# bbc/vc2-reference

Measured on AMD Instinct MI355X. Metric: Mpixels/s encode+decode, UHD-1 10-bit HQ_ConstQ, higher is better.
Workload: dtype int32; 1 GPU; BASELINE cfg2: UHD-1 3840x2160 4:2:2 10-bit HQ_ConstQ DD97 depth 4, -u 1 -a 2 -q 16 -S 2; streams=1, parallelism=frame-parallel x1, no collective

## Files before the change

include/vc2hip.h:

```cpp
#ifndef VC2HIP_H
#define VC2HIP_H

#include <stddef.h>
#include <stdint.h>

#ifdef __cplusplus
extern "C" {
#endif
#if defined(__GNUC__)
#pragma GCC visibility push(default)
#endif

typedef struct vc2hip_ctx vc2hip_ctx;

enum { VC2HIP_DD97 = 0, VC2HIP_LEGALL = 1, VC2HIP_DD137 = 2, VC2HIP_HAAR0 = 3,
       VC2HIP_HAAR1 = 4, VC2HIP_FIDELITY = 5, VC2HIP_DAUB97 = 6 };
enum { VC2HIP_CF444 = 0, VC2HIP_CF422 = 1, VC2HIP_CF420 = 2 };
enum { VC2HIP_HQ_CONSTQ = 0, VC2HIP_HQ_CBR = 1, VC2HIP_LD = 2, VC2HIP_HQ_CAPPED = 3 };
#define VC2HIP_CAP_Q_TOP 115

enum {
  VC2HIP_OK = 0,
  VC2HIP_EINVAL = -1,
  VC2HIP_EQINDEX = -2,
  VC2HIP_ESCALAR = -3,
  VC2HIP_ECBR_TOOBIG = -4,
  VC2HIP_ECBR_LEN = -5,
  VC2HIP_ECBR_WRONG = -6,
  VC2HIP_EBOUNDED = -7,
  VC2HIP_ELD_TOOBIG = -8,
  VC2HIP_ECAP = -9,
  VC2HIP_ESTREAM = -10,
  VC2HIP_ECODE32 = -11,
  VC2HIP_ESYNTAX = -12,
  VC2HIP_EHIP = -100
};

int vc2hip_create(int device, vc2hip_ctx **out);
#define VC2HIP_FLAG_STORE32         0x001u
#define VC2HIP_FLAG_NO_STREAM       0x002u
#define VC2HIP_FLAG_NO_PAIR         0x004u
#define VC2HIP_FLAG_NO_BANDPLANES   0x008u
#define VC2HIP_FLAG_NO_HEADS        0x010u
#define VC2HIP_FLAG_NO_CBR_INDEX    0x020u
#define VC2HIP_FLAG_GENERIC_DWT     0x040u
#define VC2HIP_FLAG_SINGLE_PASS_VBR 0x080u
#define VC2HIP_FLAG_CBR_GENERAL     0x100u
#define VC2HIP_FLAG_LD_DIAGONALS    0x200u
#define VC2HIP_FLAG_PLANES8_ALWAYS  0x400u
#define VC2HIP_FLAG_PLANES8_NEVER   0x800u
#define VC2HIP_FLAG_TWO_PASS_VBR    0x1000u
#define VC2HIP_FLAG_CAP_GENERAL     0x2000u
int vc2hip_create_with_flags(int device, unsigned flags, vc2hip_ctx **out);
int vc2hip_create_on_stream(int device, void *hip_stream, vc2hip_ctx **out);
int vc2hip_create_on_stream_with_flags(int device, void *hip_stream, unsigned flags, vc2hip_ctx **out);
void vc2hip_destroy(vc2hip_ctx *ctx);
const char *vc2hip_last_error(const vc2hip_ctx *ctx);
const char *vc2hip_error_string(int code);
int vc2hip_sync(vc2hip_ctx *ctx);

int vc2hip_padded_size(int size, int depth);
int vc2hip_slice_size_is_valid(int depth, int len_luma, int len_chroma, int n_size);
int vc2hip_quant_matrix(int kernel, int depth, int32_t *out);
int vc2hip_slice_bytes(int y_slices, int x_slices, int total_bytes, int scalar, int32_t *out);

int vc2hip_dwt_forward(vc2hip_ctx *ctx, const int32_t *in, int h, int w, int kernel, int depth,
                       int32_t *out);
int vc2hip_dwt_inverse(vc2hip_ctx *ctx, const int32_t *in, int ph, int pw, int kernel, int depth,
                       int32_t *out, int h, int w);
int vc2hip_quantise_np(vc2hip_ctx *ctx, const int32_t *coef, int ph, int pw, int depth,
                       const int32_t *qidx, int ys, int xs, const int32_t *qmatrix, int32_t *out);
int vc2hip_dequantise_np(vc2hip_ctx *ctx, const int32_t *q, int ph, int pw, int depth,
                         const int32_t *qidx, int ys, int xs, const int32_t *qmatrix, int32_t *out);
int vc2hip_dequantise_ld(vc2hip_ctx *ctx, const int32_t *q, int ph, int pw, int depth,
                         const int32_t *qidx, int ys, int xs, const int32_t *qmatrix, int32_t *out);

int vc2hip_quantise_ld(vc2hip_ctx *ctx, const int32_t *coef, int ph, int pw, int depth,
                       const int32_t *qidx, int ys, int xs, const int32_t *qmatrix, int32_t *out);

typedef struct {
  int luma_h, luma_w;
  int chroma_h, chroma_w;
  int depth;
  int y_slices, x_slices;
} vc2hip_geom;

int vc2hip_hq_pack(vc2hip_ctx *ctx, const int32_t *y, const int32_t *u, const int32_t *v,
                   const vc2hip_geom *g, const int32_t *qidx, int prefix, int scalar,
                   const int32_t *cbr_slice_bytes, uint8_t *out, size_t cap, size_t *out_len);
int vc2hip_hq_unpack(vc2hip_ctx *ctx, const uint8_t *in, size_t len, const vc2hip_geom *g,
                     int prefix, int scalar, int32_t *y, int32_t *u, int32_t *v, int32_t *qidx,
                     size_t *consumed);
int vc2hip_ld_unpack(vc2hip_ctx *ctx, const uint8_t *in, size_t len, const vc2hip_geom *g,
                     const int32_t *slice_bytes, int32_t *y, int32_t *u, int32_t *v,
                     int32_t *qidx, size_t *consumed);
int vc2hip_ld_pack(vc2hip_ctx *ctx, const int32_t *y, const int32_t *u, const int32_t *v,
                   const vc2hip_geom *g, const int32_t *qidx, const int32_t *slice_bytes,
                   uint8_t *out, size_t cap, size_t *out_len);
int vc2hip_ld_qindices(vc2hip_ctx *ctx, const int32_t *y, const int32_t *u, const int32_t *v,
                       const vc2hip_geom *g, const int32_t *qmatrix, const int32_t *slice_bytes,
                       int32_t *qidx);
int vc2hip_cbr_qindices(vc2hip_ctx *ctx, const int32_t *y, const int32_t *u, const int32_t *v,
                        const vc2hip_geom *g, const int32_t *qmatrix, const int32_t *slice_bytes,
                        int scalar, int32_t *qidx);

// ... 55 lines not shown
  int packing;
  int little_endian, lsb_justified;
  size_t pitch[2];
  size_t plane_offset[2];
  size_t picture_stride;
} vc2hip_packed_format;
int vc2hip_set_packed_format(vc2hip_ctx *ctx, const vc2hip_packed_format *pf);
size_t vc2hip_packed_picture_bytes(const vc2hip_picture_format *fmt, const vc2hip_packed_format *pf);
int vc2hip_encode_batch_dev(vc2hip_ctx *ctx, const void *d_raw, int n,
                            const vc2hip_picture_format *fmt, const vc2hip_coding_params *cp,
                            void *d_payload, size_t payload_stride, uint64_t *d_lens);
int vc2hip_decode_batch_dev(vc2hip_ctx *ctx, const void *d_payload, size_t payload_stride,
                            const uint64_t *d_lens, int n, const vc2hip_picture_format *fmt,
                            const vc2hip_coding_params *cp, void *d_raw_out);
int vc2hip_decode_reduced_batch_dev(vc2hip_ctx *ctx, const void *d_payload, size_t payload_stride,
                                    const uint64_t *d_lens, int n, const vc2hip_picture_format *fmt,
                                    const vc2hip_coding_params *cp, int drop_levels, void *d_raw_out);
int vc2hip_encode_recon_batch_dev(vc2hip_ctx *ctx, const void *d_raw, int n,
                                  const vc2hip_picture_format *fmt, const vc2hip_coding_params *cp,
                                  void *d_payload, size_t payload_stride, uint64_t *d_lens,
                                  void *d_recon, uint64_t *d_sse, int32_t *d_qidx);
int vc2hip_encode_fields_batch_dev(vc2hip_ctx *ctx, const void *d_frames, int n_frames,
                                   const vc2hip_picture_format *frame_fmt, int top_field_first,
                                   const vc2hip_coding_params *cp, void *d_payload, size_t payload_stride,
                                   uint64_t *d_lens);
int vc2hip_decode_fields_batch_dev(vc2hip_ctx *ctx, const void *d_payload, size_t payload_stride,
                                   const uint64_t *d_lens, int n_frames, const vc2hip_picture_format *frame_fmt,
                                   int top_field_first, const vc2hip_coding_params *cp, void *d_frames_out);

typedef struct {
  int major_version;
  uint32_t first_picture_number;
  uint32_t prev_parse_offset;
  int end_of_sequence;
} vc2hip_stream_params;

int vc2hip_picture_header(const vc2hip_coding_params *cp, int major_version, uint32_t picture_number,
                          uint8_t *out, size_t cap, size_t *len);
int vc2hip_stream_write_dev(vc2hip_ctx *ctx, const void *d_payload, size_t payload_stride, const uint64_t *d_lens, int n,
                            const vc2hip_coding_params *cp, const vc2hip_stream_params *sp,
                            uint8_t *d_stream, size_t cap, uint64_t *d_stream_len);
int vc2hip_stream_write_fragments_dev(vc2hip_ctx *ctx, const void *d_payload, size_t payload_stride,
                                      const uint64_t *d_lens, int n, const vc2hip_coding_params *cp,
                                      const vc2hip_stream_params *sp, int fragment_length,
                                      uint8_t *d_stream, size_t cap, uint64_t *d_stream_len,
                                      uint64_t *d_unit_offsets, size_t unit_cap, uint64_t *d_unit_count);
int vc2hip_stream_read_dev(vc2hip_ctx *ctx, const uint8_t *d_stream, size_t len, int n,
                           const vc2hip_coding_params *cp, const vc2hip_stream_params *sp,
                           void *d_payload, size_t payload_stride, uint64_t *d_lens,
                           uint32_t *d_picture_numbers, uint64_t *d_consumed);

int vc2hip_band_plane_bits(const vc2hip_ctx *ctx);

#define VC2HIP_DWT_TILE   0
#define VC2HIP_DWT_FAST   1
#define VC2HIP_DWT_STREAM 2
#define VC2HIP_DWT_PAIR   3
#define VC2HIP_DWT_PLANE  4
typedef struct {
  int inverse;
  int level;
  int levels;
  int family;
  int edge;
  int store_bits;
  int segments;
  int tail;
  int small_gather;
  int pictures;
  int band_planes;
} vc2hip_dwt_launch;
int vc2hip_dwt_launches(const vc2hip_ctx *ctx, vc2hip_dwt_launch *out, int cap);

int vc2hip_profile_enable(vc2hip_ctx *ctx, int on);
int vc2hip_profile_only(vc2hip_ctx *ctx, const char *name);
int vc2hip_profile_count(vc2hip_ctx *ctx);
int vc2hip_profile_get(vc2hip_ctx *ctx, int i, const char **name, int *launches, double *total_ms);
int vc2hip_profile_reset(vc2hip_ctx *ctx);

#if defined(__GNUC__)
#pragma GCC visibility pop
#endif
#ifdef __cplusplus
}
#endif
#endif
```

vc2-reference_amd/csrc/vc2hip_api.hip:

```cpp
#include <math.h>
#include <stdio.h>
#include <stdlib.h>
#include <string.h>

#include <algorithm>
#include <string>
#include <map>
#include <mutex>
#include <utility>
#include <vector>

#include "vc2hip_internal.h"

void vc2_upload_tables_slices(const QuantTables &t, hipStream_t s);
int vc2_halo_x(int kernel);
int vc2_halo_y(int kernel);
void vc2_upload_vlc_lut(hipStream_t s);
void vc2_upload_unpack_lut(hipStream_t s);
bool vc2_slice_index_supported(int prefix, int scalar);
size_t vc2_pack_lds_bytes(int prefix, int scalar);
int vc2_pack_image_mode(int prefix, int scalar);
void vc2_upload_tables_fast(const QuantTables &t, hipStream_t s);
bool vc2_fast_level_applicable(LevelParams &p);
int vc2_launch_forward_fast(Launcher &L, int kernel, bool first, const LevelParams &p, int n, bool store16, hipStream_t s);
// ... 86 lines not shown
#endif
}
void vc2_prof_break(Launcher &L) { (void)L; }

struct Buf {
  void *p = nullptr;
  size_t cap = 0;
};
enum { B_RAW, B_STORE, B_STOREW, B_LL0, B_LLW, B_QIDX, B_SLOTS, B_SIZES, B_OFFS, B_LENS, B_PAYLOAD,
       B_INDEX, B_PLANE, B_PLANE2, B_CBRB, B_CBRO, B_QM, B_UNITS, B_SEGS,
       B_FRAGS, B_FRAGPIC, B_FRAGJUMP,
       B_RSTORE, B_RSTOREW,
       B_PLANE_QM,
       B_CAPTAB,
       B_PKIN, B_PKOUT,
       B_COUNT };

struct vc2hip_ctx {
  int device = 0;
  hipStream_t stream = nullptr;
  bool own_stream = false;
  bool follows_caller = false;
  unsigned *d_err = nullptr;
  unsigned *h_err = nullptr;
  Buf buf[B_COUNT];
  Launcher L;
  std::string err;
  int cbr_key[5] = {-1, -1, -1, -1, -1};
  uint64_t cbr_total = 0;
  int plane_qm_key[2] = {-1, -1};
  int debug_skip = 0;
  bool two_pass_vbr = true;
  bool force_two_pass_vbr = false;
#ifndef VC2_ONE_PASS_MIN_PICTURES
#define VC2_ONE_PASS_MIN_PICTURES 112
#endif
  bool force_generic = false;
  bool allow_store16 = true;
  bool allow_planes = true;
  int planes8_mode = 0;
  bool planes8_on = false;
  unsigned long long *d_stat = nullptr;
  unsigned long long *h_stat = nullptr;
  hipEvent_t stat_ev = nullptr;
  bool stat_pending = false, stat_was8 = false, stat_seen = false;
  int stat_n = 0;
  int stat_n_total = 0;
  int last_plane_bits = 0;
  std::vector<vc2hip_dwt_launch> dwt_rec;
  bool dwt_rec_stale = true;
  double stat_samples = 0;
  int ld_batch = 1;
  bool allow_heads = true;
  bool allow_cbr_index = true;
  bool allow_stream = true;
  bool allow_pair = true;
  bool cbr_general = false;
  bool cap_general = false;
  bool ld_diagonals = false;
  unsigned flags = 0;
  std::vector<vc2hip_ctx *> lanes;
  bool in_split = false;
  hipEvent_t fork_ev = nullptr;
  std::vector<hipEvent_t> join_ev;
  bool lanes_pending = false;
  struct Range { const uint8_t *lo, *hi; };
  enum { LANE_RANGES = 5 };
  struct LaneUse { Range r[LANE_RANGES], w[LANE_RANGES]; bool valid = false; };
  std::vector<LaneUse> lane_use;
  std::vector<ProfEntry> merged;
  struct Flight {
    vc2hip_ctx *lane = nullptr;
    bool open = false, encode = false;
    uint8_t *payload = nullptr;
    size_t cap = 0;
    unsigned long long *h_len = nullptr;
  };
  Flight flight[VC2HIP_MAX_INFLIGHT];
  int flight_next = 0;
  vc2hip_sample_layout layout = {};
  bool has_layout = false, layout_bypass = false;
  vc2hip_packed_format packed = {};
  bool has_packed = false;
};

static const char *code_text(int code) {
  switch (code) {
    case VC2HIP_OK: return "ok";
    case VC2HIP_EINVAL: return "invalid argument";
    case VC2HIP_EQINDEX: return "quantization index exceeds maximum implemented value.";
    case VC2HIP_ESCALAR: return "Slice scalar is too small, consider using a larger slice scalar.";
    case VC2HIP_ECBR_TOOBIG: return "SliceIO, HQ CBR mode: Too many bytes for the slice";
    case VC2HIP_ECBR_LEN: return "Slice component length exceeds 1 byte when divided by slice size scalar. See above for suggestions to prevent this.";
    case VC2HIP_ECBR_WRONG: return "SliceIO, HQ CBR mode: Wrong number of bytes for a slice";
    case VC2HIP_EBOUNDED: return "Attempt to write beyond end of bounded write";
    case VC2HIP_ELD_TOOBIG: return "SliceIO, LD mode: Too many bytes for the U and V slices";
    case VC2HIP_ECAP: return "output buffer too small";
    case VC2HIP_ESTREAM: return "truncated or malformed slice data";
    case VC2HIP_ECODE32: return "quantised coefficient magnitude exceeds 65534 (outside the 32-bit exp-Golomb code domain)";
    case VC2HIP_ESYNTAX: return "VC-2 stream syntax error";
    case VC2HIP_EHIP: return "HIP runtime error";
  }
  return "unknown error";
}
extern "C" const char *vc2hip_error_string(int code) { return code_text(code); }

// ... 68 lines not shown
  const int n = ys * xs;
  int num = total_bytes / scalar - 4 * n, den = n;
  const int g = gcd_i(num, den);
  if (g) { num /= g; den /= g; }
  const int ratio = num / den, rem = num - ratio * den;
  int residue = 0;
  for (int i = 0; i < n; ++i) {
    residue += rem;
    if (residue < den) out[i] = ratio * scalar + 4;
    else { out[i] = (ratio + 1) * scalar + 4; residue -= den; }
  }
  return 0;
}
static void make_tables(QuantTables &t) {
  for (int q = 0; q < 120; ++q) {
    const uint64_t base = 1ull << (q / 4);
    uint64_t f;
    switch (q % 4) {
      case 0: f = 4 * base; break;
      case 1: f = (503829 * base + 52958) / 105917; break;
      case 2: f = (665857 * base + 58854) / 117708; break;
      default: f = (440253 * base + 32722) / 65444; break;
    }
    t.qf[q] = (int32_t)(uint32_t)f;
    t.off[q] = q == 0 ? 1 : (q == 1 ? 2 : (int32_t)(((uint32_t)t.qf[q] + 1u)) / 2);
    t.magic[q] = 0;
    t.shift[q] = 0;
    if (t.qf[q] > 1) {
      const uint64_t d = (uint64_t)t.qf[q];
      int l = 0;
      while ((1ull << l) < d) ++l;
      t.magic[q] = (uint32_t)((((1ull << l) - d) << 32) / d + 1);
      t.shift[q] = l - 1;
    }
    const double r = 4.0 / (double)(uint32_t)t.qf[q];
    float up = (float)r;
    if ((double)up < r) up = nextafterf(up, INFINITY);
    t.inv4[q] = up;
  }
}

static int create_common(int device, hipStream_t stream, bool own, vc2hip_ctx **out, unsigned flags = 0) {
  if (!out) return VC2HIP_EINVAL;
  *out = nullptr;
  int n = 0;
  if (hipGetDeviceCount(&n) != hipSuccess || device < 0 || device >= n) return VC2HIP_EHIP;
  vc2hip_ctx *c = new vc2hip_ctx;
  c->device = device;
#ifdef VC2HIP_ABLATE
  {
    static const struct { const char *name; unsigned flag; } env[] = {
      {"VC2HIP_STORE32", VC2HIP_FLAG_STORE32}, {"VC2HIP_NO_STREAM", VC2HIP_FLAG_NO_STREAM}, {"VC2HIP_NO_PAIR", VC2HIP_FLAG_NO_PAIR},
      {"VC2HIP_NO_BANDPLANES", VC2HIP_FLAG_NO_BANDPLANES}, {"VC2HIP_NO_HEADS", VC2HIP_FLAG_NO_HEADS},
      {"VC2HIP_NO_CBR_INDEX", VC2HIP_FLAG_NO_CBR_INDEX}, {"VC2HIP_GENERIC_DWT", VC2HIP_FLAG_GENERIC_DWT},
      {"VC2HIP_SINGLE_PASS_VBR", VC2HIP_FLAG_SINGLE_PASS_VBR}, {"VC2HIP_TWO_PASS_VBR", VC2HIP_FLAG_TWO_PASS_VBR}, {"VC2HIP_CBR_GENERAL", VC2HIP_FLAG_CBR_GENERAL}, {"VC2HIP_CAP_GENERAL", VC2HIP_FLAG_CAP_GENERAL},
      {"VC2HIP_PLANES8_ALWAYS", VC2HIP_FLAG_PLANES8_ALWAYS}, {"VC2HIP_PLANES8_NEVER", VC2HIP_FLAG_PLANES8_NEVER}};
    for (const auto &e : env) { const char *v = getenv(e.name); if (v && v[0] == '1') flags |= e.flag; }
    { const char *v = getenv("VC2HIP_LD_ROWS"); if (v && v[0] == '0') flags |= VC2HIP_FLAG_LD_DIAGONALS; }
    { const char *e = getenv("VC2HIP_DEBUG_SKIP"); c->debug_skip = e ? atoi(e) : 0; }
  }
#endif
  c->force_generic = (flags & VC2HIP_FLAG_GENERIC_DWT) != 0;
  c->allow_store16 = !(flags & VC2HIP_FLAG_STORE32);
  c->allow_stream = !(flags & VC2HIP_FLAG_NO_STREAM);
  c->allow_pair = !(flags & VC2HIP_FLAG_NO_PAIR);
  c->allow_planes = !(flags & VC2HIP_FLAG_NO_BANDPLANES);
  c->planes8_mode = (flags & VC2HIP_FLAG_PLANES8_NEVER) ? 2 : (flags & VC2HIP_FLAG_PLANES8_ALWAYS) ? 1 : 0;
  c->allow_heads = !(flags & VC2HIP_FLAG_NO_HEADS);
  c->allow_cbr_index = !(flags & VC2HIP_FLAG_NO_CBR_INDEX);
  c->two_pass_vbr = !(flags & VC2HIP_FLAG_SINGLE_PASS_VBR);
  c->force_two_pass_vbr = (flags & VC2HIP_FLAG_TWO_PASS_VBR) != 0;
  c->cbr_general = (flags & VC2HIP_FLAG_CBR_GENERAL) != 0;
  c->cap_general = (flags & VC2HIP_FLAG_CAP_GENERAL) != 0;
  c->ld_diagonals = (flags & VC2HIP_FLAG_LD_DIAGONALS) != 0;
  c->flags = flags;
  if (hipSetDevice(device) != hipSuccess) { delete c; return VC2HIP_EHIP; }
  if (own) { if (hipStreamCreateWithFlags(&stream, hipStreamNonBlocking) != hipSuccess) { delete c; return VC2HIP_EHIP; } }
  c->stream = stream;
  c->own_stream = own;
  c->follows_caller = !own;
  if (hipMalloc((void **)&c->d_err, 256 + 4096) != hipSuccess ||
     
      hipHostMalloc((void **)&c->h_err, VC2_ERRBLK_COPY) != hipSuccess ||
      hipMalloc((void **)&c->d_stat, 64) != hipSuccess || hipHostMalloc((void **)&c->h_stat, 64 * 8) != hipSuccess ||
      hipEventCreateWithFlags(&c->stat_ev, hipEventDisableTiming) != hipSuccess) { delete c; return VC2HIP_EHIP; }
  (void)hipMemsetAsync(c->d_stat, 0, 64, c->stream);
  (void)hipMemsetAsync(c->d_err, 0, sizeof(unsigned), c->stream);
  QuantTables t;
  make_tables(t);
  vc2_upload_tables(t, c->stream);
  vc2_upload_tables_slices(t, c->stream);
  vc2_upload_tables_fast(t, c->stream);
  vc2_upload_tables_pair(t, c->stream);
  vc2_upload_tables_stream(t, c->stream);
  vc2_upload_tables_recon(t, c->stream);
  vc2_upload_vlc_lut(c->stream);
  vc2_upload_unpack_lut(c->stream);
  if (hipStreamSynchronize(c->stream) != hipSuccess) { delete c; return VC2HIP_EHIP; }
  *out = c;
  return VC2HIP_OK;
}
extern "C" int vc2hip_create(int device, vc2hip_ctx **out) { return create_common(device, nullptr, true, out); }
extern "C" int vc2hip_create_with_flags(int device, unsigned flags, vc2hip_ctx **out) { return create_common(device, nullptr, true, out, flags); }
extern "C" int vc2hip_create_on_stream(int device, void *s, vc2hip_ctx **out) { return create_common(device, (hipStream_t)s, false, out); }
extern "C" int vc2hip_create_on_stream_with_flags(int device, void *s, unsigned flags, vc2hip_ctx **out) {
  return create_common(device, (hipStream_t)s, false, out, flags);
}
extern "C" void vc2hip_destroy(vc2hip_ctx *c) {
  if (!c) return;
  (void)hipSetDevice(c->device);
  (void)hipStreamSynchronize(c->stream);
  for (vc2hip_ctx *l : c->lanes) if (l != c) vc2hip_destroy(l);
  for (auto &f : c->flight) { if (f.lane) vc2hip_destroy(f.lane); if (f.h_len) (void)hipHostFree(f.h_len); }
  for (hipEvent_t e : c->join_ev) (void)hipEventDestroy(e);
  if (c->fork_ev) (void)hipEventDestroy(c->fork_ev);
  c->L.collect();
  for (auto e : c->L.pool) (void)hipEventDestroy(e);
  for (auto &b : c->buf) if (b.p) (void)hipFree(b.p);
  if (c->d_err) (void)hipFree(c->d_err);
  if (c->h_err) (void)hipHostFree(c->h_err);
  if (c->h_stat) (void)hipHostFree(c->h_stat);
// ... 440 lines not shown
      const size_t e = (size_t)(g.c[c].ph >> l) * (g.c[c].pw >> l);
      ll.p[l][c] = (char *)base + off * elem_bytes;
      ll.w[l][c] = wide ? wide + off : nullptr;
      ll.stride[l][c] = (long long)e;
      off += (e * n + 7) & ~(size_t)7;
    }
}
static void ll_layout(const Geom &g, int n, int32_t *base, LLPlanes &ll) { ll_layout(g, n, base, 4, nullptr, ll); }

static void record_dwt(vc2hip_ctx *c, bool inverse, int level, int levels, int family, bool edge, bool s16, int segments, int tail,
                       bool small_gather, int n, int band_planes = 0) {
  if (c->dwt_rec_stale) { c->dwt_rec.clear(); c->dwt_rec_stale = false; }
  vc2hip_dwt_launch r;
  r.inverse = inverse; r.level = level; r.levels = levels; r.family = family; r.edge = edge; r.store_bits = s16 ? 16 : 32;
  r.segments = segments; r.tail = tail; r.small_gather = small_gather; r.pictures = n; r.band_planes = band_planes;
  c->dwt_rec.push_back(r);
}

static int band_plane_bits(const LevelParams &p) {
  for (int k = 0; k < 3; ++k) if (p.bp_base[k] >= 0) return p.bp8 ? 8 : 16;
  return 0;
}

static void fill_level(LevelParams &p, const Geom &g, int level, int kernel, const int32_t *qm) {
  const int D = g.depth, Lv = D - level;
  p.band = 3 * (Lv - 1) + 1;
  p.ys = g.ys; p.xs = g.xs; p.slice_coefs = g.slice_coefs;
  const int hx = vc2_halo_x(kernel), hy = vc2_halo_y(kernel);
  for (int c = 0; c < 3; ++c) {
    const CompGeom &cg = g.c[c];
    p.in_h[c] = cg.ph >> level; p.in_w[c] = cg.pw >> level;
    p.pic_h[c] = cg.h; p.pic_w[c] = cg.w;
    p.coef_off[c] = cg.coef_off;
    p.rec_stride[c] = g.slice_coefs;
    if (cg.ph == 0) { p.tiles_x[c] = p.tiles_y[c] = 0; p.fh[c] = p.fw[c] = 2; p.tsy[c] = p.tsx[c] = 1; continue; }
    p.fh[c] = cg.sh >> level; p.fw[c] = cg.sw >> level;
    int tsy = 1, tsx = 1;
    while (tsy * 2 * p.fh[c] <= 64 && tsy * 2 <= g.ys) tsy *= 2;
    while (tsx * 2 * p.fw[c] <= 128 && tsx * 2 <= g.xs) tsx *= 2;
    while ((size_t)(tsy * p.fh[c] + 2 * hy) * (tsx * p.fw[c] + 2 * hx) * 4 > 150 * 1024) {
      if (tsx > 1) tsx /= 2; else if (tsy > 1) tsy /= 2; else break;
    }
    p.tsy[c] = tsy; p.tsx[c] = tsx;
    p.tiles_y[c] = (g.ys + tsy - 1) / tsy;
    p.tiles_x[c] = (g.xs + tsx - 1) / tsx;
    p.band_n[c] = (p.fh[c] / 2) * (p.fw[c] / 2);
    p.band_off[c] = p.band_n[c];
  }
  for (int b = 0; b < 3 * D + 1; ++b) p.qmatrix[b] = qm ? qm[b] : 0;
}

static int run_forward(vc2hip_ctx *c, const Geom &g, int kernel, int n, const void *const src[3],
                       const RawPlane src_l[3], bool src_raw, const vc2hip_picture_format *f,
                       void *store, const LLPlanes &ll, bool s16 = false, int32_t *store_wide = nullptr) {
  auto level_params = [&](LevelParams &p, int level) {
    memset(&p, 0, sizeof p);
    fill_level(p, g, level, kernel, nullptr);
    p.store = store; p.store_stride = (long long)g.ys * g.xs * g.slice_coefs;
    p.store_wide = store_wide;
    p.err = c->d_err;
    p.ll_to_store = (level == g.depth - 1);
    const bool first = (level == 0) && src_raw;
    for (int k = 0; k < 3; ++k) {
      if (level == 0) { p.plane[k] = (void *)src[k]; p.plane_stride[k] = src_l[k].stride; }
      else { p.plane[k] = ll.p[level][k]; p.plane_wide[k] = ll.w[level][k]; p.plane_stride[k] = ll.stride[level][k]; }
      p.ll[k] = ll.p[level + 1][k]; p.ll_wide[k] = ll.w[level + 1][k]; p.ll_stride[k] = ll.stride[level + 1][k];
    }
    if (first) {
      for (int k = 0; k < 3; ++k) { p.raw_pitch[k] = src_l[k].pitch; p.field_step[k] = src_l[k].field_step; }
      p.field_shift = src_l[0].field_shift;
      p.word_bytes = f->word_bytes;
      const int lsb = src_l[0].lsb;
      p.sample_shift = lsb ? 0 : 8 * f->word_bytes - f->bit_depth;
      p.sample_offset = 1 << (f->bit_depth - 1);
      const int cd = f->chroma_bit_depth ? f->chroma_bit_depth : f->bit_depth;
      p.sample_shift_c = lsb ? 0 : 8 * f->word_bytes - cd;
      p.sample_offset_c = 1 << (cd - 1);
      p.sample_bits = f->bit_depth; p.sample_bits_c = cd;
      p.sample_mask = f->bit_depth < 32 ? (1u << f->bit_depth) - 1 : ~0u;
      p.sample_mask_c = cd < 32 ? (1u << cd) - 1 : ~0u;
      p.sample_le = src_l[0].le;
      p.perm_rd = src_l[0].le ? VC2_PERM_RD_LE : VC2_PERM_RD_BE;
    }
  };
  for (int level = 0; level < g.depth; ++level) {
    LevelParams p;
    level_params(p, level);
    const bool first = (level == 0) && src_raw;
    if (!c->force_generic && c->allow_stream && c->allow_pair && level + 1 < g.depth) {
      PairParams pp;
      memset(&pp, 0, sizeof pp);
      pp.a = p;
      pp.a.debug_skip = c->debug_skip;
      level_params(pp.b, level + 1);
      const size_t lds = vc2_pair_applicable(pp, kernel, first, false, s16, n);
      if (lds) {
        int rc = vc2_launch_forward_pair(c->L, kernel, first, pp, n, s16, lds, c->stream);
        if (rc) return set_err(c, rc, "invalid wavelet kernel");
        record_dwt(c, false, level, 2, VC2HIP_DWT_PAIR, first, s16, pp.a.st_segmax, 0, false, n);
        ++level;
        continue;
      }
    }
    LevelParams pf = p;
    pf.debug_skip = c->debug_skip;
    if (!c->force_generic && c->allow_stream) {
      LevelParams ps = p;
      const size_t lds = vc2_stream_level_applicable(ps, kernel, first, false, s16, n);
      if (lds) {
        int rc = vc2_launch_forward_stream(c->L, kernel, first, ps, n, s16, lds, c->stream);
        if (rc) return set_err(c, rc, "invalid wavelet kernel");
        record_dwt(c, false, level, 1, VC2HIP_DWT_STREAM, first, s16, ps.st_segmax, ps.st_tail, false, n);
        continue;
      }
    }
    if (!c->force_generic && vc2_fast_level_applicable(pf)) {
      int rc = vc2_launch_forward_fast(c->L, kernel, first, pf, n, s16, c->stream);
      if (rc) return set_err(c, rc, "invalid wavelet kernel");
      record_dwt(c, false, level, 1, VC2HIP_DWT_FAST, first, s16, 0, 0, false, n);
      continue;
    }
    if (s16) return set_err(c, VC2HIP_EINVAL, "internal: 16-bit store without the fast level kernels");
    if (vc2_level_lds_bytes(kernel, p) > 160 * 1024) return set_err(c, VC2HIP_EINVAL, "slice too large for one LDS tile");
    int rc = vc2_launch_forward_level(c->L, kernel, first, p, n, c->stream);
    if (rc) return set_err(c, rc, "invalid wavelet kernel");
    record_dwt(c, false, level, 1, VC2HIP_DWT_TILE, first, false, 0, 0, false, n);
  }
  return VC2HIP_OK;
}

static int run_inverse(vc2hip_ctx *c, const Geom &g, int kernel, int n, void *store, const int32_t *qidx,
                       const int32_t *qm, bool dequant, bool ll_ready, const LLPlanes &ll, void *const dst[3],
                       const RawPlane *dst_l, bool dst_raw, const vc2hip_picture_format *f,
                       bool s16 = false, int32_t *store_wide = nullptr, const BandPlanes *bp = nullptr,
                       long long store_stride = 0, unsigned *stream_mask = nullptr, const HeadSplit *hs = nullptr, int head_level = 1 << 30,
                       unsigned *fast_mask = nullptr, unsigned *tail_mask = nullptr, int norm_shift = 0, int level_base = 0) {
  if (tail_mask) *tail_mask = 0;
  if (stream_mask) *stream_mask = 0;
  if (fast_mask) *fast_mask = 0;
  auto level_params = [&](LevelParams &p, int level) {
    memset(&p, 0, sizeof p);
    fill_level(p, g, level, kernel, qm);
    if (hs && level >= head_level)
      for (int k = 0; k < 3; ++k) if (g.c[k].ph) { p.rec_stride[k] = hs->n[k]; p.coef_off[k] = (int)hs->base[k]; }
    p.store = store; p.store_stride = store_stride ? store_stride : (long long)g.ys * g.xs * g.slice_coefs;
    for (int k = 0; k < 3; ++k) p.bp_base[k] = (bp && level < bp->levels && g.c[k].ph) ? bp->base[k][level] : -1;
    p.bp8 = bp && level < bp->levels && bp->bytes8;
    p.store_wide = store_wide;
    p.qidx = qidx; p.err = c->d_err; p.dequant = dequant;
    p.ll_from_store = (level == g.depth - 1) && !ll_ready;
    const bool fin = (level == 0) && dst_raw;
    for (int k = 0; k < 3; ++k) {
      if (level == 0) { p.plane[k] = dst ? dst[k] : nullptr; p.plane_stride[k] = dst_l ? dst_l[k].stride : 0; }
      else { p.plane[k] = ll.p[level][k]; p.plane_wide[k] = ll.w[level][k]; p.plane_stride[k] = ll.stride[level][k]; }
      p.ll[k] = ll.p[level + 1][k]; p.ll_wide[k] = ll.w[level + 1][k]; p.ll_stride[k] = ll.stride[level + 1][k];
    }
// ... 105 lines not shown
    const long long ps = (long long)cg.ph * cg.pw;
    int32_t *pl = d_plane + off;
    off += (size_t)ps * n;
    vc2_launch_plane_ingest(c->L, src[k], ss[k], cg.h, cg.w, f->word_bytes, k && f->chroma_bit_depth ? f->chroma_bit_depth : f->bit_depth, pl, ps,
                            cg.ph, cg.pw, n, c->stream);
    const int rc = vc2_launch_plane_transform(c->L, kernel, pl, ps, cg.ph, cg.pw, g.depth, false, n, c->stream);
    if (rc) return set_err(c, rc, "invalid wavelet kernel");
    record_dwt(c, false, 0, g.depth, VC2HIP_DWT_PLANE, false, false, 0, 0, false, n);
    for (int p = 0; p < n; ++p)
      vc2_launch_plane_to_store(c->L, pl + (size_t)p * ps, cg.ph, cg.pw, g.depth, g.ys, g.xs,
                                d_store + (size_t)p * g.ys * g.xs * g.slice_coefs, g.slice_coefs, cg.coef_off, c->stream);
  }
  return VC2HIP_OK;
}
static int plane_inverse(vc2hip_ctx *c, const Geom &g, int kernel, int n, const int32_t *d_store, const int32_t *d_q, const int32_t *qm,
                         void *const dst[3], const RawPlane ds[3], const vc2hip_picture_format *f, const LLPlanes *ll = nullptr,
                         int norm_shift = 0, int level_base = 0) {
  int32_t *d_plane;
  int *d_qm;
  NEED(c, B_PLANE, plane_elems(g) * n * 4, d_plane);
  NEED(c, B_PLANE_QM, 256, d_qm);
  const int key[2] = {kernel, g.depth | (g.depth + level_base) << 8};
  if (memcmp(key, c->plane_qm_key, sizeof key)) {
    c->plane_qm_key[0] = -1;
    HIPCHK(c, hipMemcpyAsync(d_qm, qm, (size_t)(3 * g.depth + 1) * 4, hipMemcpyHostToDevice, c->stream));
    HIPCHK(c, hipStreamSynchronize(c->stream));
    memcpy(c->plane_qm_key, key, sizeof key);
  }
  const int ns = g.ys * g.xs;
  size_t off = 0;
  for (int k = 0; k < 3; ++k) {
    const CompGeom &cg = g.c[k];
    if (!cg.ph) continue;
    const long long ps = (long long)cg.ph * cg.pw;
    int32_t *pl = d_plane + off;
    off += (size_t)ps * n;
    for (int p = 0; p < n; ++p)
      vc2_launch_store_to_plane(c->L, d_store + (size_t)p * ns * g.slice_coefs, g.slice_coefs, cg.coef_off, pl + (size_t)p * ps, cg.ph,
                                cg.pw, g.depth, g.ys, g.xs, d_q + (size_t)p * ns, d_qm, 1, c->d_err, c->stream);
    if (ll) vc2_launch_ll_into_plane(c->L, (const int32_t *)ll->p[g.depth][k], ll->stride[g.depth][k], cg.ph >> g.depth, cg.pw >> g.depth, pl, ps,
                                     cg.pw, g.depth, n, c->stream);
    const int rc = vc2_launch_plane_transform(c->L, kernel, pl, ps, cg.ph, cg.pw, g.depth, true, n, c->stream);
    if (rc) return set_err(c, rc, "invalid wavelet kernel");
    record_dwt(c, true, level_base, g.depth, VC2HIP_DWT_PLANE, false, false, 0, 0, false, n);
    vc2_launch_plane_emit(c->L, pl, ps, cg.pw, dst[k], ds[k], cg.h, cg.w, f->word_bytes, f->bit_depth, n, c->stream, norm_shift);
  }
  return VC2HIP_OK;
}

static void fill_comp_arrays(const Geom &g, int n[3], int off[3], int n0[3]) {
  for (int c = 0; c < 3; ++c) { n[c] = g.c[c].sh * g.c[c].sw; off[c] = g.c[c].coef_off; n0[c] = g.c[c].n0 ? g.c[c].n0 : 1; }
}

static int run_pack(vc2hip_ctx *c, const Geom &g, int n, const void *store, const int32_t *d_qidx,
                    const int32_t *qm, bool quantise, int prefix, int scalar, const int32_t *d_cbr_bytes,
                    const uint32_t *d_cbr_offs, uint64_t cbr_total, uint8_t *d_payload, long long stride,
                    unsigned long long *d_lens, bool s16 = false, const int32_t *store_wide = nullptr) {
  const int ns = g.ys * g.xs;
  PackParams p;
  memset(&p, 0, sizeof p);
  p.store = store; p.store_stride = (long long)ns * g.slice_coefs;
  p.store16 = s16; p.store_wide = store_wide;
  p.qidx = d_qidx; p.n_slices = ns; p.slice_coefs = g.slice_coefs;
  fill_comp_arrays(g, p.comp_n, p.comp_off, p.comp_n0);
  p.depth = g.depth; p.prefix = prefix; p.scalar = scalar;
  for (int b = 0; b < 3 * g.depth + 1; ++b) p.qmatrix[b] = qm ? qm[b] : 0;
  p.err = c->d_err; p.quantise = quantise;
  p.payload = d_payload; p.payload_stride = stride;
  const bool gimg = vc2_pack_image_mode(prefix, scalar) < 0;
  if (d_cbr_bytes && !gimg) {
    p.cbr_bytes = d_cbr_bytes; p.cbr_offsets = d_cbr_offs;
    vc2_launch_pack(c->L, p, n, c->stream);
    vc2_launch_fill_u64(c->L, d_lens, cbr_total, (size_t)n, c->stream);
    return VC2HIP_OK;
  }
  const bool one_pass = !gimg && !d_cbr_bytes &&
                        (!c->two_pass_vbr || (!c->force_two_pass_vbr && n >= VC2_ONE_PASS_MIN_PICTURES && vc2_pack_one_pass_default(p)));
  if (one_pass) {
    const long long lb_stride = (long long)((ns + 3) / 4) + 8;
    unsigned long long *lb;
    NEED(c, B_SIZES, (size_t)n * lb_stride * 8, lb);
    HIPCHK(c, hipMemsetAsync(lb, 0, (size_t)n * lb_stride * 8, c->stream));
    vc2_prof_break(c->L);
    p.lookback = lb; p.lookback_stride = lb_stride; p.lens = d_lens;
    vc2_launch_pack(c->L, p, n, c->stream);
    return VC2HIP_OK;
  }
  const int slot = (int)((max_slice_bytes(prefix, scalar) + (gimg ? 8 : 0) + 15) & ~(size_t)15);
  uint8_t *slots; uint32_t *sizes, *offs;
  const int spt_room = (gimg || d_cbr_bytes) ? 0 : vc2_pack_slices_per_tile(p);
  const size_t slot_count = spt_room ? (size_t)((ns + spt_room - 1) / spt_room) * spt_room : (size_t)ns;
  NEED(c, B_SLOTS, (size_t)n * slot_count * slot + 32, slots);
  NEED(c, B_SIZES, (size_t)n * ns * 4, sizes);
  NEED(c, B_OFFS, (size_t)n * ns * 4, offs);
  p.slots = slots; p.slot_bytes = slot; p.sizes = sizes;
  if (d_cbr_bytes) { p.cbr_bytes = d_cbr_bytes; p.cbr_offsets = d_cbr_offs; }
  const int spt = (gimg || d_cbr_bytes) ? 0 : vc2_pack_slices_per_tile(p);
  p.tile_slices = spt;
  vc2_launch_pack(c->L, p, n, c->stream);
  if (spt) {
    const int nt = (ns + spt - 1) / spt;
    vc2_launch_scan_sizes(c->L, sizes, offs, d_lens, nt, n, c->stream);
    vc2_launch_compact(c->L, slots, spt * slot, sizes, offs, d_payload, stride, nt, n, c->stream);
    return VC2HIP_OK;
  }
  vc2_launch_scan_sizes(c->L, sizes, offs, d_lens, ns, n, c->stream);
  vc2_launch_compact(c->L, slots, slot, sizes, offs, d_payload, stride, ns, n, c->stream);
  return VC2HIP_OK;
}

static int one_plane_geom(Geom &g, int ph, int pw, int depth, int ys, int xs) {
  int phs[3] = {ph, 0, 0}, pws[3] = {pw, 0, 0};
  return make_geom(g, phs, pws, phs, pws, depth, ys, xs);
}

extern "C" int vc2hip_dwt_forward(vc2hip_ctx *c, const int32_t *in, int h, int w, int kernel, int depth,
                                  int32_t *out) {
  if (!c || !in || !out || h < 1 || w < 1 || depth < 1 || depth > VC2_MAX_DEPTH) return set_err(c, VC2HIP_EINVAL);
  if (kernel < 0 || kernel > 6) return set_err(c, VC2HIP_EINVAL, "invalid wavelet kernel");
  ENTER(c);
  const int ph = vc2hip_padded_size(h, depth), pw = vc2hip_padded_size(w, depth);
  Geom g;
  int rc = one_plane_geom(g, ph, pw, depth, ph >> depth, pw >> depth);
  if (rc) return set_err(c, rc);
  std::vector<int32_t> padded((size_t)ph * pw);
  for (int y = 0; y < ph; ++y)
    for (int x = 0; x < pw; ++x) padded[(size_t)y * pw + x] = in[(size_t)(y < h ? y : h - 1) * w + (x < w ? x : w - 1)];
  int32_t *d_plane, *d_store, *d_ll;
  const size_t pb = (size_t)ph * pw * 4;
  NEED(c, B_PLANE, pb, d_plane);
  NEED(c, B_STORE, pb, d_store);
  NEED(c, B_LL0, ll_bytes(g, 1) + 16, d_ll);
  LLPlanes ll;
  ll_layout(g, 1, d_ll, ll);
  HIPCHK(c, hipMemcpyAsync(d_plane, padded.data(), pb, hipMemcpyHostToDevice, c->stream));
  const void *src[3] = {d_plane, nullptr, nullptr};
  const RawPlane ss[3] = {{(long long)ph * pw, 0, 0, 0}, {}, {}};
  rc = run_forward(c, g, kernel, 1, src, ss, false, nullptr, d_store, ll);
  if (rc) return rc;
  vc2_launch_store_to_plane(c->L, d_store, g.slice_coefs, 0, d_plane, ph, pw, depth, g.ys, g.xs, nullptr, nullptr, 0,
                            c->d_err, c->stream);
  HIPCHK(c, hipMemcpyAsync(out, d_plane, pb, hipMemcpyDeviceToHost, c->stream));
  return vc2hip_sync(c);
}

extern "C" int vc2hip_dwt_inverse(vc2hip_ctx *c, const int32_t *in, int ph, int pw, int kernel, int depth,
                                  int32_t *out, int h, int w) {
  if (!c || !in || !out || depth < 1 || depth > VC2_MAX_DEPTH || h < 1 || w < 1 || h > ph || w > pw) return set_err(c, VC2HIP_EINVAL);
  if (kernel < 0 || kernel > 6) return set_err(c, VC2HIP_EINVAL, "invalid wavelet kernel");
  if (ph % (1 << depth) || pw % (1 << depth)) return set_err(c, VC2HIP_EINVAL);
// ... 597 lines not shown
                     const int32_t *d_cb, bool check, const LdEncParams *ld);

extern "C" int vc2hip_encode_recon_batch_dev(vc2hip_ctx *c, const void *d_raw, int n, const vc2hip_picture_format *f,
                                             const vc2hip_coding_params *cp, void *d_payload, size_t payload_stride, uint64_t *d_lens,
                                             void *d_recon, uint64_t *d_sse, int32_t *d_qidx) {
  if (!c || !d_raw || n < 1 || !f || !cp) return set_err(c, VC2HIP_EINVAL);
  if (!d_payload && !d_recon && !d_sse && !d_qidx) return set_err(c, VC2HIP_EINVAL, "no output asked for");
  if (d_sse && !d_recon) return set_err(c, VC2HIP_EINVAL, "d_sse needs d_recon");
  if ((d_payload != nullptr) != (payload_stride != 0) || (d_payload != nullptr) != (d_lens != nullptr))
    return set_err(c, VC2HIP_EINVAL, "d_payload, payload_stride and d_lens: all or none");
  if (((size_t)d_raw | (size_t)d_payload | (size_t)d_recon | payload_stride) & 15 || (((size_t)d_lens | (size_t)d_sse) & 7) || ((size_t)d_qidx & 3))
    return set_err(c, VC2HIP_EINVAL, "device buffers and the payload stride must be 16-byte aligned");
  Geom ge;
  if (picture_geom(ge, f, cp, false)) return set_err(c, VC2HIP_EINVAL);
  RawLayout lay;
  if (int rc = batch_layout(c, f, lay)) return rc;
  const size_t rb = lay.stride, span = (size_t)(n - 1) * lay.stride + lay.extent;
  const int ns = ge.ys * ge.xs;
  const uint8_t *raw8 = (const uint8_t *)d_raw;
  uint8_t *rec8 = (uint8_t *)d_recon;
  if (d_recon) {
    if (rec8 < raw8 + span && raw8 < rec8 + span)
      return set_err(c, VC2HIP_EINVAL, "d_recon overlaps d_raw (the squared error reads the input after the reconstruction is written)");
    if (f->chroma_bit_depth && f->chroma_bit_depth != f->bit_depth)
      return set_err(c, VC2HIP_EINVAL, "the decoder has one bit depth: chroma_bit_depth must be 0 or bit_depth with d_recon");
    Geom gd;
    if (picture_geom(gd, f, cp, true)) return set_err(c, VC2HIP_EINVAL);
    for (int k = 0; k < 3; ++k)
      if (gd.c[k].ph != ge.c[k].ph || gd.c[k].pw != ge.c[k].pw)
        return set_err(c, VC2HIP_EINVAL, "the decoder's padded chroma planes differ from the encoder's: no decoder shows this picture");
  }
  if (c->lanes.size() > 1 && n > 1 && !c->in_split) {
    uint8_t *pay8 = (uint8_t *)d_payload;
    auto rng = [](const void *p, size_t first, size_t count, size_t each) {
      const uint8_t *q = (const uint8_t *)p;
      return q ? vc2hip_ctx::Range{q + first * each, q + (first + count) * each} : vc2hip_ctx::Range{nullptr, nullptr};
    };
    return split_batch(c, n,
      [&](int first, int count, vc2hip_ctx::LaneUse &u) {
        u.r[0] = rng(d_raw, first, count, rb);
        u.w[0] = rng(d_payload, first, count, payload_stride); u.w[1] = rng(d_lens, first, count, 8);
        u.w[2] = rng(d_recon, first, count, rb); u.w[3] = rng(d_sse, first, count, 24); u.w[4] = rng(d_qidx, first, count, (size_t)ns * 4);
      },
      [&](vc2hip_ctx *l, int first, int count) {
        return vc2hip_encode_recon_batch_dev(l, raw8 + (size_t)first * rb, count, f, cp, pay8 ? pay8 + (size_t)first * payload_stride : nullptr,
                                             payload_stride, d_lens ? d_lens + first : nullptr, rec8 ? rec8 + (size_t)first * rb : nullptr,
                                             d_sse ? d_sse + 3 * (size_t)first : nullptr, d_qidx ? d_qidx + (size_t)first * ns : nullptr);
      });
  }
  const ReconOut ro = {d_recon, d_sse, d_qidx};
  return encode_batch_common(c, d_raw, 1, 1, n, f, cp, d_payload, payload_stride, d_lens, &ro);
}

static int encode_batch_common(vc2hip_ctx *c, const void *d_raw, int fields, int top_first, int n, const vc2hip_picture_format *f,
                               const vc2hip_coding_params *cp, void *d_payload, size_t payload_stride, uint64_t *d_lens,
                               const ReconOut *ro) {
  if (cp->mode != VC2HIP_HQ_CONSTQ && cp->mode != VC2HIP_HQ_CBR && cp->mode != VC2HIP_LD && cp->mode != VC2HIP_HQ_CAPPED) return set_err(c, VC2HIP_EINVAL);
  if (cp->mode == VC2HIP_HQ_CAPPED && (cp->q_index < 0 || cp->q_index > VC2_CAP_Q_TOP || cp->compressed_bytes < 1))
    return set_err(c, VC2HIP_EINVAL, "HQ_CAPPED: q_index 0 .. 115, compressed_bytes >= 1");
  if (cp->kernel < 0 || cp->kernel > 6) return set_err(c, VC2HIP_EINVAL, "invalid wavelet kernel");
  if (cp->mode != VC2HIP_LD && (cp->scalar < 1 || cp->prefix < 0)) return set_err(c, VC2HIP_EINVAL);
  Geom g;
  int rc = picture_geom(g, f, cp, false);
  if (rc) return set_err(c, rc);
  {
    vc2hip_picture_format fb = *f;
    fb.height = f->height * fields;
    RawLayout lay;
    if ((rc = batch_layout(c, &fb, lay))) return rc;
  }
  ENTER(c);
  const int ns = g.ys * g.xs;
  int32_t qm[VC2_MAX_BANDS];
  if ((rc = vc2hip_quant_matrix(cp->kernel, cp->depth, qm))) return set_err(c, rc);
  const bool s16 = cp->mode != VC2HIP_LD && use_store16(c, g, cp->kernel);
  int32_t *d_store, *d_ll, *d_q, *d_storew = nullptr, *d_llw = nullptr;
  NEED(c, B_STORE, (size_t)n * ns * g.slice_coefs * 4, d_store);
  NEED(c, B_LL0, ll_bytes(g, n) + 16, d_ll);
  if (s16) {
    NEED(c, B_STOREW, (size_t)n * ns * g.slice_coefs * 4, d_storew);
    NEED(c, B_LLW, ll_bytes(g, n) + 16, d_llw);
  }
  NEED(c, B_QIDX, (size_t)n * ns * 4, d_q);
  LLPlanes ll;
  ll_layout(g, n, d_ll, s16 ? 2 : 4, d_llw, ll);
  const void *src[3]; RawPlane ss[3];
  RawView in;
  {
    vc2hip_picture_format fb = *f;
    fb.height = f->height * fields;
    if ((rc = raw_view(c, &fb, n / fields, d_raw, B_PKIN, in))) return rc;
  }
  view_convert(c, in, false);
  view_planes(in, f, fields, top_first, src, ss);
  if (needs_plane_path(c, g, cp->kernel)) {
    if ((rc = plane_forward(c, g, cp->kernel, n, src, ss, f, d_store))) return rc;
  } else if ((rc = run_forward(c, g, cp->kernel, n, src, ss, true, f, d_store, ll, s16, d_storew))) return rc;
  int32_t *d_cb = nullptr; uint32_t *d_co = nullptr; uint64_t total = 0;
  if (cp->mode == VC2HIP_LD) {
    const int key[5] = {g.ys, g.xs, cp->compressed_bytes, 1, -7};
    if (memcmp(key, c->cbr_key, sizeof key) || !c->buf[B_CBRB].p) {
      std::vector<int32_t> sb(ns);
      vc2hip_slice_bytes(g.ys, g.xs, cp->compressed_bytes, 1, sb.data());
      if ((rc = ld_offsets_upload(c, sb.data(), ns, &d_cb, &d_co, &total))) return rc;
      memcpy(c->cbr_key, key, sizeof key);
      c->cbr_total = total;
    }
    d_cb = (int32_t *)c->buf[B_CBRB].p; d_co = (uint32_t *)c->buf[B_CBRO].p; total = c->cbr_total;
    if (d_payload && total > payload_stride) return set_err(c, VC2HIP_ECAP);
    LdEncParams p;
    c->ld_batch = n;
    if ((rc = fill_ld_enc(c, p, g, d_store, d_q, qm, ll, d_cb, d_co, cp->compressed_bytes / ns + 5, (uint8_t *)d_payload,
                          (long long)payload_stride))) return rc;
    p.search = 1;
    vc2_launch_ld_quantise(c->L, p, n, c->stream);
    if (d_payload) {
      vc2_launch_ld_pack(c->L, p, n, c->stream);
      vc2_launch_fill_u64(c->L, (unsigned long long *)d_lens, total, (size_t)n, c->stream);
    }
    return ro ? run_recon(c, g, cp, n, f, qm, false, d_store, nullptr, d_q, ll, in, *ro, d_cb, !d_payload, &p) : VC2HIP_OK;
  }
  if (cp->mode == VC2HIP_HQ_CBR) {
      const int key[5] = {g.ys, g.xs, cp->compressed_bytes, cp->scalar, cp->prefix};
    if (memcmp(key, c->cbr_key, sizeof key) || !c->buf[B_CBRB].p) {
      std::vector<int32_t> sb(ns);
      vc2hip_slice_bytes(g.ys, g.xs, cp->compressed_bytes, cp->scalar, sb.data());
      if ((rc = cbr_offsets_upload(c, sb.data(), ns, cp->prefix, &d_cb, &d_co, &total))) return rc;
      memcpy(c->cbr_key, key, sizeof key);
      c->cbr_total = total;
    }
    d_cb = (int32_t *)c->buf[B_CBRB].p; d_co = (uint32_t *)c->buf[B_CBRO].p; total = c->cbr_total;
    if (d_payload && total > payload_stride) return set_err(c, VC2HIP_ECAP);
    CbrParams p;
    memset(&p, 0, sizeof p);
    p.store = d_store; p.store_stride = (long long)ns * g.slice_coefs; p.qidx = d_q; p.slice_bytes = d_cb;
    p.store16 = s16; p.store_wide = d_storew;
    p.n_slices = ns; p.slice_coefs = g.slice_coefs;
    fill_comp_arrays(g, p.comp_n, p.comp_off, p.comp_n0);
    p.scalar = cp->scalar; p.err = c->d_err;
    p.general_only = c->cbr_general;
    for (int b = 0; b < 3 * g.depth + 1; ++b) p.qmatrix[b] = qm[b];
    p.n_bands = 3 * g.depth + 1;
    vc2_launch_cbr(c->L, p, n, c->stream);
  } else if (cp->mode == VC2HIP_HQ_CAPPED) {
    if (d_payload && payload_stride < vc2hip_max_payload_bytes(f, cp)) return set_err(c, VC2HIP_ECAP);
    CapParams p;
    memset(&p, 0, sizeof p);
    NEED(c, B_CAPTAB, (size_t)n * VC2_CAP_ROW * 8, p.table);
    HIPCHK(c, hipMemsetAsync(p.table, 0, (size_t)n * VC2_CAP_ROW * 8, c->stream));
    p.s.store = d_store; p.s.store_stride = (long long)ns * g.slice_coefs; p.s.qidx = d_q;
    p.s.store16 = s16; p.s.store_wide = d_storew;
    p.s.n_slices = ns; p.s.slice_coefs = g.slice_coefs;
    fill_comp_arrays(g, p.s.comp_n, p.s.comp_off, p.s.comp_n0);
    p.s.scalar = cp->scalar; p.s.err = c->d_err;
    p.s.general_only = c->cap_general;
    for (int b = 0; b < 3 * g.depth + 1; ++b) p.s.qmatrix[b] = qm[b];
    p.s.n_bands = 3 * g.depth + 1;
    p.prefix = cp->prefix; p.floor = cp->q_index; p.cap = (unsigned long long)cp->compressed_bytes;
    vc2_launch_cap(c->L, p, n, c->stream);
  } else {
    if (d_payload && payload_stride < vc2hip_max_payload_bytes(f, cp)) return set_err(c, VC2HIP_ECAP);
    vc2_launch_fill_i32(c->L, d_q, cp->q_index, (size_t)n * ns, c->stream);
  }
  if (d_payload && (rc = run_pack(c, g, n, d_store, d_q, qm, true, cp->prefix, cp->scalar, d_cb, d_co, total, (uint8_t *)d_payload,
                                  (long long)payload_stride, (unsigned long long *)d_lens, s16, d_storew))) return rc;
  return ro ? run_recon(c, g, cp, n, f, qm, s16, d_store, d_storew, d_q, ll, in, *ro, d_cb, !d_payload, nullptr) : VC2HIP_OK;
}

static int run_recon(vc2hip_ctx *c, const Geom &g, const vc2hip_coding_params *cp, int n, const vc2hip_picture_format *f, const int32_t *qm,
                     bool s16, int32_t *d_store, int32_t *d_storew, int32_t *d_q, const LLPlanes &ll, const RawView &in, const ReconOut &ro,
                     const int32_t *d_cb, bool check, const LdEncParams *ld) {
  const int ns = g.ys * g.xs;
  int rc;
  if (ro.qidx) HIPCHK(c, hipMemcpyAsync(ro.qidx, d_q, (size_t)n * ns * 4, hipMemcpyDeviceToDevice, c->stream));
  const void *dstc[3]; RawPlane ds[3];
  RawView out;
  if ((rc = raw_view(c, f, n, ro.recon, B_PKOUT, out))) return rc;
  view_planes(out, f, 1, 1, dstc, ds);
  void *dst[3] = {(void *)dstc[0], (void *)dstc[1], (void *)dstc[2]};
  const bool plane_path = needs_plane_path(c, g, cp->kernel);
  if (ld) {
    if (check) vc2_launch_ld_check(c->L, *ld, n, c->stream);
    if (ro.recon) {
      LdLl3Params lp;
      lp.store = d_store; lp.store_stride = (long long)ns * g.slice_coefs; lp.slice_coefs = g.slice_coefs;
      lp.ys = g.ys; lp.xs = g.xs; lp.qidx = d_q; lp.qm0 = qm[0]; lp.err = c->d_err;
      for (int k = 0; k < 3; ++k) {
        lp.coef_off[k] = g.c[k].coef_off; lp.llh[k] = g.c[k].ph >> g.depth; lp.llw[k] = g.c[k].pw >> g.depth;
        lp.ll_plane[k] = (int32_t *)ll.p[g.depth][k]; lp.ll_stride[k] = ll.stride[g.depth][k];
      }
      if (!vc2_launch_ld_ll3(c->L, lp, n, c->stream))
        for (int k = 0; k < 3; ++k)
          vc2_launch_ld_ll(c->L, d_store, (long long)ns * g.slice_coefs, g.slice_coefs, g.c[k].coef_off, g.c[k].n0,
                           g.c[k].ph >> g.depth, g.c[k].pw >> g.depth, g.ys, g.xs, d_q, qm[0], (int32_t *)ll.p[g.depth][k],
                           ll.stride[g.depth][k], n, c->d_err, c->stream);
      if (plane_path) rc = plane_inverse(c, g, cp->kernel, n, d_store, d_q, qm, dst, ds, f, &ll);
      else rc = run_inverse(c, g, cp->kernel, n, d_store, d_q, qm, true, true, ll, dst, ds, true, f);
      if (rc) return rc;
    }
  } else if (ro.recon || check) {
    DecoderLayout lay;
    plan_decoder_layout(c, g, cp->kernel, n, false, qm, dst, ds, f, s16, plane_path, lay);
    int32_t *d_rs = nullptr, *d_rsw = nullptr;
    if (ro.recon) {
      NEED(c, B_RSTORE, (size_t)n * (size_t)lay.sstride * (s16 ? 2 : 4), d_rs);
      if (s16) NEED(c, B_RSTOREW, (size_t)n * (size_t)lay.sstride * 4, d_rsw);
    }
    RequantParams p;
    memset(&p, 0, sizeof p);
    p.src = d_store; p.src_wide = d_storew; p.src_stride = (long long)ns * g.slice_coefs;
    p.dst = d_rs; p.dst_wide = d_rsw; p.dst_stride = lay.sstride;
    p.store16 = s16; p.qidx = d_q; p.n_slices = ns; p.slice_coefs = g.slice_coefs; p.xs = g.xs;
    fill_comp_arrays(g, p.comp_n, p.comp_off, p.comp_n0);
    p.n_bands = 3 * g.depth + 1;
    for (int b = 0; b < p.n_bands; ++b) p.qmatrix[b] = qm[b];
    p.bp = lay.bp; p.hs = lay.hs;
    p.check = check; p.scalar = cp->scalar; p.cbr_bytes = d_cb; p.err = c->d_err;
    vc2_launch_requantise(c->L, p, n, c->stream);
// ... 200 lines not shown
      HIPCHK(c, hipMemcpyAsync(c->h_stat + 1, d_lens, (size_t)c->stat_n * 8, hipMemcpyDeviceToHost, c->stream));
      HIPCHK(c, hipEventRecord(c->stat_ev, c->stream));
      c->stat_pending = true;
    }
  } else {
    int32_t *d_sb; uint32_t *d_so; uint64_t total;
    const int key[5] = {g.ys, g.xs, cp->compressed_bytes, 1, -7};
    if (memcmp(key, c->cbr_key, sizeof key) || !c->buf[B_CBRB].p) {
      std::vector<int32_t> sb(ns);
      vc2hip_slice_bytes(g.ys, g.xs, cp->compressed_bytes, 1, sb.data());
      if ((rc = ld_offsets_upload(c, sb.data(), ns, &d_sb, &d_so, &total))) return rc;
      memcpy(c->cbr_key, key, sizeof key);
      c->cbr_total = total;
    }
    d_sb = (int32_t *)c->buf[B_CBRB].p; d_so = (uint32_t *)c->buf[B_CBRO].p; total = c->cbr_total;
    if (total > payload_stride) return set_err(c, VC2HIP_ESTREAM);
    LdUnpackParams p;
    fill_ld_unpack(p, g, (const uint8_t *)d_payload, (long long)payload_stride, d_sb, d_so, d_store, d_q, c->d_err);
    unsigned *d_shifted; uint32_t *d_starts;
    NEED(c, B_SIZES, (size_t)n * 4, d_shifted);
    NEED(c, B_OFFS, (size_t)n * ns * 4, d_starts);
    int flag_fill = 0;
#ifdef VC2HIP_ABLATE
    if (getenv("VC2HIP_DEBUG_LD_REDO")) flag_fill = 1;
#endif
    HIPCHK(c, hipMemsetAsync(d_shifted, flag_fill, (size_t)n * 4, c->stream));
    vc2_prof_break(c->L);
    p.lens = (const unsigned long long *)d_lens; p.shifted = d_shifted; p.starts = d_starts;
    vc2_launch_ld_unpack(c->L, p, n, c->stream);
    vc2_launch_ld_walk(c->L, p, n, c->stream);
    p.redo = 1;
    vc2_launch_ld_unpack(c->L, p, n, c->stream);
    LdLl3Params lp;
    lp.store = d_store; lp.store_stride = (long long)ns * g.slice_coefs; lp.slice_coefs = g.slice_coefs;
    lp.ys = g.ys; lp.xs = g.xs; lp.qidx = d_q; lp.qm0 = qm[0]; lp.err = c->d_err;
    for (int k = 0; k < 3; ++k) {
      lp.coef_off[k] = g.c[k].coef_off; lp.llh[k] = g.c[k].ph >> g.depth; lp.llw[k] = g.c[k].pw >> g.depth;
      lp.ll_plane[k] = (int32_t *)ll.p[g.depth][k]; lp.ll_stride[k] = ll.stride[g.depth][k];
    }
    if (!vc2_launch_ld_ll3(c->L, lp, n, c->stream))
    for (int k = 0; k < 3; ++k)
      vc2_launch_ld_ll(c->L, d_store, (long long)ns * g.slice_coefs, g.slice_coefs, g.c[k].coef_off, g.c[k].n0,
                       g.c[k].ph >> g.depth, g.c[k].pw >> g.depth, g.ys, g.xs, d_q, qm[0], (int32_t *)ll.p[g.depth][k],
                       ll.stride[g.depth][k], n, c->d_err, c->stream);
  }
  if (plane_path) rc = plane_inverse(c, g, cp->kernel, n, d_store, d_q, qm, dst, ds, f, ld ? &ll : nullptr, norm_shift, drop);
  else rc = run_inverse(c, g, cp->kernel, n, d_store, d_q, qm, true, ld, ll, dst, ds, true, f, s16, d_storew, &bp, sstride, nullptr,
                        hs.n[0] ? &hs : nullptr, head_level, nullptr, nullptr, norm_shift, drop);
  if (!rc) view_convert(c, out, true);
  return rc;
}

extern "C" int vc2hip_band_plane_bits(const vc2hip_ctx *c) { return c ? c->last_plane_bits : 0; }

namespace {
struct HeaderBits {
  uint8_t *out;
  size_t cap, pos = 0;
  unsigned cache = 0;
  int cached = 0;
  void bit(unsigned b) {
    cache = (cache << 1) | (b & 1);
    if (++cached == 8) { if (pos < cap) out[pos] = (uint8_t)cache; ++pos; cache = 0; cached = 0; }
  }
  void uvlc(uint32_t v) {
    const unsigned long long x = (unsigned long long)v + 1;
    int top = 63;
    while (!(x >> top & 1)) --top;
    for (int i = top - 1; i >= 0; --i) { bit(0); bit((unsigned)(x >> i) & 1); }
    bit(1);
  }
  void align() { while (cached) bit(0); }
};
bool stream_cp_ok(const vc2hip_coding_params *cp) {
  if (!cp || cp->kernel < 0 || cp->kernel > 6 || cp->depth < 0 || cp->y_slices < 1 || cp->x_slices < 1) return false;
  if (cp->mode == VC2HIP_LD) return cp->compressed_bytes > 0;
  return (cp->mode == VC2HIP_HQ_CONSTQ || cp->mode == VC2HIP_HQ_CBR || cp->mode == VC2HIP_HQ_CAPPED) && cp->prefix >= 0 && cp->scalar >= 1;
}
void stream_ab(const vc2hip_coding_params *cp, uint32_t *a, uint32_t *b) {
  if (cp->mode != VC2HIP_LD) { *a = (uint32_t)cp->prefix; *b = (uint32_t)cp->scalar; return; }
  const int ns = cp->y_slices * cp->x_slices, g = gcd_i(cp->compressed_bytes, ns);
  *a = (uint32_t)(cp->compressed_bytes / g);
  *b = (uint32_t)(ns / g);
}
}

extern "C" int vc2hip_picture_header(const vc2hip_coding_params *cp, int major_version, uint32_t picture_number, uint8_t *out,
                                     size_t cap, size_t *len) {
  if (!stream_cp_ok(cp) || major_version < 1 || !len || (cap && !out)) return VC2HIP_EINVAL;
  uint32_t a, b;
  stream_ab(cp, &a, &b);
  HeaderBits w{out, cap};
  for (int i = 24; i >= 0; i -= 8) for (int k = 7; k >= 0; --k) w.bit(picture_number >> (i + k));
  w.uvlc((uint32_t)cp->kernel);
  w.uvlc((uint32_t)cp->depth);
  if (major_version >= 3) { w.bit(0); w.bit(0); }
  w.uvlc((uint32_t)cp->x_slices);
  w.uvlc((uint32_t)cp->y_slices);
  w.uvlc(a);
  w.uvlc(b);
  w.bit(0);
  w.align();
  *len = w.pos;
  return w.pos > cap ? VC2HIP_ECAP : VC2HIP_OK;
}

// ... 403 lines not shown
```

vc2-reference_amd/csrc/vc2hip_dwt_pair.hip:

```cpp
#include <stdio.h>
#include <stdlib.h>

#include <algorithm>
#include <map>
#include <mutex>
#include <tuple>
#include <type_traits>
#include <vector>

#include "vc2hip_internal.h"
#include "vc2hip_store.h"
#include "vc2hip_wavelets.h"

void vc2_prof_begin(Launcher &L, const char *name, hipStream_t s);
void vc2_prof_end(Launcher &L, hipStream_t s);

__constant__ QuantTables c_qsp;
void vc2_upload_tables_pair(const QuantTables &t, hipStream_t s) {
  (void)hipMemcpyToSymbolAsync(HIP_SYMBOL(c_qsp), &t, sizeof t, 0, hipMemcpyHostToDevice, s);
}

namespace {

#ifndef VC2_PAIR_NT
#define VC2_PAIR_NT 1
#endif
#include "vc2hip_stream_eng.h"

__device__ __forceinline__ void pair_prio(int mode, int prio0, int block) {
  if (mode == 1) { prio_turn(prio0 + block); return; }
  const int t = mode == 2 ? block : block >> (mode - 2);
  if ((prio0 + t) & 1) __builtin_amdgcn_s_setprio(3);
  else __builtin_amdgcn_s_setprio(0);
}

template <int V> using IC = std::integral_constant<int, V>;
template <bool V> using BC = std::integral_constant<bool, V>;

template <int K> constexpr bool pair_kernel() {
  if constexpr (K == VC2HIP_FIDELITY || K == VC2HIP_DAUB97) return false;
  else return reach_fits<K, 2>() && reach_fits<K, 4>() && WT<K>::nsteps == 2;
}
template <int K> constexpr int pair_halo() { return halo_lanes<K, 4>() + halo_lanes<K, 2>(); }
constexpr int fdiv2(int v) { return v >= 0 ? v / 2 : -((-v + 1) / 2); }

#ifndef VC2_PAIR_WPE
#define VC2_PAIR_WPE 2
#endif
template <int K> constexpr int pair_wpe() { return K == VC2HIP_DD137 ? 2 : VC2_PAIR_WPE; }
#ifndef VC2_PAIR_PF
#define VC2_PAIR_PF 2
#endif
constexpr int PFP = VC2_PAIR_PF;
template <int K, bool FIRST, class ST>
__global__ __launch_bounds__(64, (pair_wpe<K>())) void k_fwd_pair(const PairParams pp) {
  using S_ = St<ST>;
  using EA = VEng<K, false, 4>;
  using EB = VEng<K, false, 2>;
  using T = VT<K, false>;
  constexpr int OFFL = T::OFFL, SD = T::sum_dmin();
  constexpr int ACC = WT<K>::accuracy;
  extern __shared__ __attribute__((aligned(16))) unsigned char smem[];
#define p pp.a
#define pb pp.b
  const int lane = threadIdx.x & 63;
  int comp, pic;
  Strip sp;
  if (!strip_of_block_h<pair_halo<K>()>(p, comp, pic, sp)) return;
  const int spl = pp.spl[comp];
  sp.nsl *= spl;
  sp.sx0 *= spl;
  ST *imgA = (ST *)smem, *imgB = (ST *)(smem + pp.img_b);
  unsigned *ring_ll = (unsigned *)(smem + pp.ring_ll);
  const int szA = pp.sz_a, szB = pp.sz_b, grpA = pp.grp_a, nll = pp.n_ll;
  const int xs = p.xs, slice_coefs = p.slice_coefs, st_prio = p.st_prio;
#ifdef VC2HIP_ABLATE
  const int dskip = p.debug_skip;
#else
  constexpr int dskip = 0;
#endif
  const int pieceA = pp.piece_a[comp], pieceB = pp.piece_b[comp];
  const int sshift = FIRST ? (comp ? p.sample_shift_c : p.sample_shift) : 0;
  const int sbits = FIRST ? (comp ? p.sample_bits_c : p.sample_bits) : 0;
  const unsigned sel_rd = p.perm_rd;
  const int bias = FIRST ? -((comp ? p.sample_offset_c : p.sample_offset) << ACC) : 0;
  const int in_h = p.in_h[comp], in_w = p.in_w[comp], npA = in_h >> 1, npB = npA >> 1;
  const int chunk = min(sp.c0 + lane, (in_w >> 3) - 1);
  const bool own = lane >= sp.lo && lane < sp.hi;
  const bool redge = sp.c0 + lane == (in_w >> 3) - 1 && lane != 63;

  const uint8_t *raw = nullptr;
  const ST *lvl = nullptr;
  const int32_t *lvl_w = nullptr;
  if constexpr (FIRST) raw = (const uint8_t *)p.plane[comp] + vc2_raw_pic_offset(p, comp, pic) + (size_t)chunk * 16;
  else {
    lvl = (const ST *)p.plane[comp] + (size_t)pic * p.plane_stride[comp] + (size_t)chunk * 8;
    if constexpr (S_::narrow) lvl_w = p.plane_wide[comp] + (size_t)pic * p.plane_stride[comp] + (size_t)chunk * 8;
  }
  const int pic_h = FIRST ? p.pic_h[comp] : in_h;
  const int rpw = FIRST ? p.raw_pitch[comp] >> 1 : in_w;
  constexpr int NQ = (FIRST || S_::narrow) ? 1 : 2;
  uint4 pf[PFP][2][NQ];
  auto fetch = [&](int m, int slot) __attribute__((always_inline)) {
#pragma unroll
    for (int h = 0; h < 2; ++h) {
      const int y = min(2 * m + h, pic_h - 1);
      if constexpr (FIRST) pf[slot][h][0] = *(const uint4 *)(raw + mul24z(y, rpw) * 2);
      else {
        const ST *q = lvl + mul24z(y, in_w);
        pf[slot][h][0] = *(const uint4 *)q;
        if constexpr (NQ == 2) pf[slot][h][1] = *(const uint4 *)(q + 4);
      }
    }
  };
  auto convert = [&](int m, int slot, int h, RowT<4> &r) __attribute__((always_inline)) {
    if constexpr (FIRST) {
      const unsigned w[4] = {pf[slot][h][0].x, pf[slot][h][0].y, pf[slot][h][0].z, pf[slot][h][0].w};
#pragma unroll
      for (int k = 0; k < 4; ++k) {
        const unsigned b = __builtin_amdgcn_perm(w[k], w[k], sel_rd);
        r[k] = (int)(__builtin_amdgcn_ubfe(b, (unsigned)sshift, (unsigned)sbits) << ACC) + bias;
        r[4 + k] = (int)(__builtin_amdgcn_ubfe(b, (unsigned)(16 + sshift), (unsigned)sbits) << ACC) + bias;
      }
    } else {
      int s[8];
      if constexpr (S_::narrow) S_::unpack8(pf[slot][h][0], lvl_w + mul24z(2 * m + h, in_w), s);
      else {
        s[0] = (int)pf[slot][h][0].x; s[1] = (int)pf[slot][h][0].y; s[2] = (int)pf[slot][h][0].z; s[3] = (int)pf[slot][h][0].w;
        s[4] = (int)pf[slot][h][NQ - 1].x; s[5] = (int)pf[slot][h][NQ - 1].y; s[6] = (int)pf[slot][h][NQ - 1].z; s[7] = (int)pf[slot][h][NQ - 1].w;
      }
#pragma unroll
      for (int k = 0; k < 4; ++k) { r[k] = (int)((unsigned)s[2 * k] << ACC); r[4 + k] = (int)((unsigned)s[2 * k + 1] << ACC); }
    }
  };

  const int bshA = p.fh[comp] >> 1, bswA = p.fw[comp] >> 1, lbshA = ilog2d(bshA), bnA = bshA * bswA;
  const int bshB = bshA >> 1, bswB = bswA >> 1, lbshB = lbshA - 1, bnB = bshB * bswB;
  const int b_last = pb.ll_to_store;
  const int run0A = p.coef_off[comp] + bnA, run0B = pb.coef_off[comp] + (b_last ? 0 : bnB);
  const int ssA = pp.ss_a[comp], ssB = pp.ss_b[comp];
  const int llps = p.st_llps[comp];
  const int si = spl == 1 ? (lane - sp.lo) >> llps : (lane - sp.lo) * spl;
  const int cl = spl == 1 ? (lane - sp.lo) & ((1 << llps) - 1) : 0;
  ST *store = (ST *)p.store + (size_t)pic * p.store_stride;
  int32_t *wide = S_::narrow ? p.store_wide + (size_t)pic * p.store_stride : nullptr;
  ST *llp = nullptr;
  int32_t *llp_w = nullptr;
  const int owB = in_w >> 2;
  if (!b_last) {
    llp = (ST *)pb.ll[comp] + (size_t)pic * pb.ll_stride[comp] + (size_t)chunk * 2;
    if constexpr (S_::narrow) llp_w = pb.ll_wide[comp] + (size_t)pic * pb.ll_stride[comp] + (size_t)chunk * 2;
  }
  const int baseA = si * ssA + cl * 4, baseB = si * ssB + cl * 2;
  auto escapes = [&](int *v, auto NBc, auto NVc, int sv, int run0, int bn, int off_r, int clv) __attribute__((always_inline)) {
    constexpr int NB = decltype(NBc)::value, NV = decltype(NVc)::value, H = NV / 2;
    if constexpr (S_::narrow) {
      int32_t *w0 = wide + mul24z(sv * xs + sp.sx0 + si, slice_coefs) + run0 + off_r + (spl == 1 ? clv : 0);
      int32_t *w1 = spl == 1 ? w0 + H : w0 + slice_coefs;
#pragma unroll
      for (int b = 0; b < NB; ++b, w0 += bn, w1 += bn)
#pragma unroll
        for (int j = 0; j < NV; ++j)
          if (!S_::fits(v[b * NV + j])) { (j < H ? w0 : w1)[j % H] = v[b * NV + j]; v[b * NV + j] = VC2_ST_SENTINEL; }
    }
  };
  auto stageA = [&](ST *img, int r, int sv, const RowT<4> &oe, const RowT<4> &oo) __attribute__((always_inline)) {
    int v[12] = {oe[4], oe[5], oe[6], oe[7], oo[0], oo[1], oo[2], oo[3], oo[4], oo[5], oo[6], oo[7]};
    if constexpr (S_::narrow) {
      int mx = v[0], mn = v[0];
#pragma unroll
      for (int j = 1; j < 12; ++j) { mx = max(mx, v[j]); mn = min(mn, v[j]); }
      if (__builtin_expect(mx > 32767 || mn < -32767, 0)) escapes(v, IC<3>(), IC<4>(), sv, run0A, bnA, r * bswA, cl * 4);
    }
    ST *d = img + baseA + r * bswA;
#pragma unroll
    for (int b = 0; b < 3; ++b, d += bnA) {
      if constexpr (S_::narrow) {
        const unsigned w0 = vc2_pack16(v[4 * b], v[4 * b + 1]), w1 = vc2_pack16(v[4 * b + 2], v[4 * b + 3]);
        if (spl == 1) *(uint2 *)d = make_uint2(w0, w1);
        else { *(unsigned *)d = w0; *(unsigned *)(d + ssA) = w1; }
      } else {
        if (spl == 1) *(int4 *)d = make_int4(v[4 * b], v[4 * b + 1], v[4 * b + 2], v[4 * b + 3]);
        else { *(int2 *)d = make_int2(v[4 * b], v[4 * b + 1]); *(int2 *)(d + ssA) = make_int2(v[4 * b + 2], v[4 * b + 3]); }
      }
    }
  };
  auto stageB = [&](ST *img, int r, int sv, const RowT<2> &oe, const RowT<2> &oo) __attribute__((always_inline)) {
    int v[8] = {oe[0], oe[1], oe[2], oe[3], oo[0], oo[1], oo[2], oo[3]};
    if constexpr (S_::narrow) {
      int mx = v[2], mn = v[2];
#pragma unroll
      for (int j = 3; j < 8; ++j) { mx = max(mx, v[j]); mn = min(mn, v[j]); }
      if (b_last) { mx = max(mx, max(v[0], v[1])); mn = min(mn, min(v[0], v[1])); }
      if (__builtin_expect(mx > 32767 || mn < -32767, 0)) {
        if (b_last) escapes(v, IC<4>(), IC<2>(), sv, run0B, bnB, r * bswB, cl * 2);
        else escapes(v + 2, IC<3>(), IC<2>(), sv, run0B, bnB, r * bswB, cl * 2);
      }
    }
    ST *d = img + baseB + r * bswB;
#pragma unroll
    for (int b = 0; b < 4; ++b) {
      if (b == 0 && !b_last) continue;
      if constexpr (S_::narrow) {
        if (spl == 1) *(unsigned *)d = vc2_pack16(v[2 * b], v[2 * b + 1]);
        else { *d = (ST)v[2 * b]; *(d + ssB) = (ST)v[2 * b + 1]; }
      } else {
        if (spl == 1) *(int2 *)d = make_int2(v[2 * b], v[2 * b + 1]);
        else { *d = (ST)v[2 * b]; *(d + ssB) = (ST)v[2 * b + 1]; }
      }
      d += bnB;
    }
  };
  auto flush = [&](const ST *img, int ss, int run0, int run_n, int piece, int sv) __attribute__((always_inline)) {
    const int epp = piece / (int)sizeof(ST), ppr = run_n / epp;
    ST *rec0 = store + mul24z(sv * xs + sp.sx0, slice_coefs) + run0;
    const bool nt = FIRST && VC2_PAIR_NT && piece == 16 && (((run0 | run_n | slice_coefs) * (int)sizeof(ST)) & 127) == 0;
    if (ppr <= 64) {
      const int spt = 64 / ppr;
      int ls = (int)((float)lane * (1.0f / (float)ppr));
      ls -= ls * ppr > lane ? 1 : 0;
      ls += (ls + 1) * ppr <= lane ? 1 : 0;
      const int e = (lane - ls * ppr) * epp;
      const ST *src = img + ls * ss + e;
      ST *dst = rec0 + mul24z(ls, slice_coefs) + e;
      const int dsrc = spt * ss;
      const size_t ddst = mul24z(spt, slice_coefs);
#pragma unroll 1
      for (int s2 = ls; s2 < sp.nsl; s2 += spt, src += dsrc, dst += ddst) {
        if (ls < spt) {
          if (piece == 16) { if (nt) st_nt(dst, *(const uint4 *)src); else *(uint4 *)dst = *(const uint4 *)src; }
          else if (piece == 8) *(uint2 *)dst = *(const uint2 *)src;
          else *(unsigned *)dst = *(const unsigned *)src;
        }
      }
    } else {
#pragma unroll 1
      for (int s2 = 0; s2 < sp.nsl; ++s2) {
        const ST *src = img + s2 * ss;
        ST *dst = rec0 + mul24z(s2, slice_coefs);
#pragma unroll 1
        for (int q = lane; q < ppr; q += 64) {
          if (piece == 16) { if (nt) st_nt(dst + q * epp, *(const uint4 *)(src + q * epp)); else *(uint4 *)(dst + q * epp) = *(const uint4 *)(src + q * epp); }
          else if (piece == 8) *(uint2 *)(dst + q * epp) = *(const uint2 *)(src + q * epp);
          else *(unsigned *)(dst + q * epp) = *(const unsigned *)(src + q * epp);
        }
      }
    }
  };

  EA engA;
  EB engB;
  engA.clear();
  engB.clear();
  const int kA = sp.kA, kB = sp.kB, kA1 = kA >> 1, kB1 = kB >> 1;
  const int want = (kA + 3 * SD) & ~1;
  const bool top = want <= 0;
  const bool bottom = kB >= npA;
  const int m0 = top ? 0 : bottom ? npA - ((npA - want + 7) & ~7) : want;
  const int mend = bottom ? npA : kB + 3 * OFFL;
  const int mload = npA - 1;
#pragma unroll
  for (int u = 0; u < PFP; ++u) fetch(min(m0 + u, mload), u);
  static_assert(8 % PFP == 0, "the prefetch ring shares the unrolled walk");
  const int sv0 = kA >> lbshA, sv1 = kB >> lbshA;
  int stA = sv0, dnA = sv0, stB = sv0, dnB = sv0, stL = kA1, dnL = kA1;
  int slotBs = 0, slotBf = 0;
  bool due = false;
  int llE[4] = {0, 0, 0, 0};
  int mb = m0;

  auto burst = [&]() __attribute__((always_inline)) {
    wave_sync();
#pragma unroll 1
    for (; stA < dnA; ++stA) if (!(dskip & 256)) flush(imgA + ((stA - sv0) & (grpA - 1)) * szA, ssA, run0A, 3 * bnA, pieceA, stA);
#pragma unroll 1
    for (; stB < dnB; ++stB) {
      if (!(dskip & 64)) flush(imgB + slotBf * szB, ssB, run0B, (b_last ? 4 : 3) * bnB, pieceB, stB);
      slotBf = slotBf == grpA ? 0 : slotBf + 1;
    }
    if (!b_last) {
#pragma unroll 1
      for (; stL < dnL; ++stL) {
        if (own && !(dskip & 128)) {
          ST *d = llp + mul24z(stL, owB);
          if constexpr (S_::narrow) *(unsigned *)d = ring_ll[(stL & (nll - 1)) * 64 + lane];
          else *(uint2 *)d = *(const uint2 *)(ring_ll + ((stL & (nll - 1)) * 64 + lane) * 2);
        }
      }
    }
    wave_sync();
    due = false;
  };
  auto deferred = [&]() __attribute__((always_inline)) { if (__builtin_expect(due, 0)) burst(); };
  auto emitB = [&](auto UBc, int k1) __attribute__((always_inline)) {
    constexpr int UB = decltype(UBc)::value;
    if (k1 >= kA1 && k1 < kB1) {
      const RowT<2> &oe = engB.template out<UB>(false), &oo = engB.template out<UB>(true);
      const int r = k1 & (bshB - 1), sv = k1 >> lbshB;
      if (!(dskip & 16)) {
        if (!b_last) {
          int a0 = oe[0], a1 = oe[1];
          if constexpr (S_::narrow) {
            if (__builtin_expect(own && (!S_::fits(a0) || !S_::fits(a1)), 0)) {
              int32_t *w = llp_w + mul24z(k1, owB);
              if (!S_::fits(a0)) { w[0] = a0; a0 = VC2_ST_SENTINEL; }
              if (!S_::fits(a1)) { w[1] = a1; a1 = VC2_ST_SENTINEL; }
            }
#if !(defined(VC2_PAIR_X) && (VC2_PAIR_X & 2))
            ring_ll[(k1 & (nll - 1)) * 64 + lane] = vc2_pack16(a0, a1);
#endif
          } else *(uint2 *)(ring_ll + ((k1 & (nll - 1)) * 64 + lane) * 2) = make_uint2((unsigned)a0, (unsigned)a1);
          dnL = k1 + 1;
        }
#if !(defined(VC2_PAIR_X) && (VC2_PAIR_X & 1))
        if (own) stageB(imgB + slotBs * szB, r, sv, oe, oo);
#endif
#if !(defined(VC2_PAIR_X) && (VC2_PAIR_X & 4))
        if (r == bshB - 1) {
          dnB = sv + 1;
          slotBs = slotBs == grpA ? 0 : slotBs + 1;
          if (sv + 1 == sv1) due = true;
        }
#endif
      }
    }
  };
  auto iter = [&](auto U0c, auto BMc, auto DRc) __attribute__((always_inline)) {
    constexpr int U0 = decltype(U0c)::value, BM = decltype(BMc)::value;
    constexpr bool DRAIN = decltype(DRc)::value;
    if constexpr (!DRAIN || U0 < OFFL) {
// ... 667 lines not shown
bool pow2p(int v) { return v > 0 && (v & (v - 1)) == 0; }
int spl_of(int fw) { return fw >= 8 ? 1 : 2; }
int ilog2h(int v) { return 31 - __builtin_clz((unsigned)v); }

int image_stride(int run_elems, int elem, int lps, int spl, int vals) {
  const int base = (run_elems * elem + 15) & ~15;
  int best = base, best_cost = 1 << 30;
  for (int pad = 0; pad <= 256; pad += 16) {
    const int ss = base + pad;
    int bank[64] = {0};
    for (int l = 0; l < 64; ++l)
      for (int q = 0; q < spl; ++q) {
        const int slice = spl == 1 ? l / lps : l * spl + q;
        const int off = spl == 1 ? (l % lps) * vals * elem : 0;
        const int bytes = std::max(4, vals / spl * elem);
        for (int b = 0; b < bytes; b += 4) ++bank[((slice * ss + off + b) >> 2) & 63];
      }
    int cost = 0;
    for (int b = 0; b < 64; ++b) cost = std::max(cost, bank[b]);
    if (cost < best_cost) { best_cost = cost; best = ss; }
  }
  return best / elem;
}

}

size_t vc2_pair_applicable(PairParams &pp, int kernel, bool edge, bool inverse, bool store16, int n_pictures) {
  PairTaps t;
  if (!pair_taps(kernel, inverse, t)) return 0;
  LevelParams &p = pp.a;
  const LevelParams &pb = pp.b;
  const int elem = store16 ? 2 : 4;
  const bool b_last = inverse ? pb.ll_from_store != 0 : pb.ll_to_store != 0;
  if (inverse && (p.bp8 || pb.bp8)) return 0;
  if (!store16) return 0;
  size_t imgA = 16, imgB = 16;
  p.st_tail = 0;
  p.st_segmax = 0;
  for (int c = 0; c < 3; ++c) {
    p.st_strips[c] = p.st_segs[c] = 0;
    pp.spl[c] = 1;
    if (p.tiles_x[c] == 0 || p.tiles_y[c] == 0) continue;
    const int w = p.in_w[c], h = p.in_h[c], fw = p.fw[c], fh = p.fh[c];
    if (w < VC2_STREAM_MIN_W || (w & 7) || (h & 3) || h < 48) return 0;
    if (edge && (p.word_bytes != 2 || p.pic_w[c] != w)) return 0;
    if (!pow2p(fw) || !pow2p(fh) || fw < 4 || fh < 4 || fw > 64 * 8) return 0;
    if (pb.fw[c] * 2 != fw || pb.fh[c] * 2 != fh || pb.in_w[c] * 2 != w || pb.in_h[c] * 2 != h) return 0;
    const int spl = fw >= 8 ? 1 : 2, lps = fw >= 8 ? fw / 8 : 1;
    const int bnA = (fh / 2) * (fw / 2), bnB = (fh / 4) * (fw / 4);
    const int runA = 3 * bnA, runB = (b_last ? 4 : 3) * bnB;
    const int pieceA = std::min(16, bnA * elem), pieceB = std::min(16, (b_last ? 4 * bnB : bnB) * elem);
    if (!inverse) {
      if (pieceA < 4 || pieceB < 4) return 0;
      if ((p.coef_off[c] * elem) % 16 || (pb.coef_off[c] * elem) % 16 || (p.slice_coefs * elem) % 16) return 0;
    } else {
      if ((p.coef_off[c] | pb.coef_off[c] | p.rec_stride[c] | pb.rec_stride[c] | bnA) & 3) return 0;
      if ((bnB & 1) && !(bnB == 1 && b_last && spl_of(fw) == 2)) return 0;
    }
    pp.piece_a[c] = pieceA;
    pp.piece_b[c] = pieceB;
    pp.spl[c] = spl;
    static const int out_cap = vc2_tune_int("VC2HIP_PAIR_OUT", 64);
    const int out = (std::min(64 - 2 * t.halo, out_cap) / lps) * lps;
    if (out < lps) return 0;
    const int nch = w / 8;
    p.st_out[c] = out;
    p.st_llps[c] = ilog2h(lps);
    p.st_strips[c] = (nch + out - 1) / out;
    const int nsl = out / lps * spl;
    pp.ss_a[c] = image_stride(runA, elem, lps, spl, 4);
    pp.ss_b[c] = (runB * elem + 15) / 16 * 16 / elem;
    imgA = std::max(imgA, (size_t)nsl * pp.ss_a[c] * elem);
    imgB = std::max(imgB, (size_t)nsl * pp.ss_b[c] * elem);
  }
  if (inverse) imgA = imgB = 0;
  imgA = (imgA + 15) & ~(size_t)15;
  imgB = (imgB + 15) & ~(size_t)15;
  int bsh_min = 1 << 20, bshb_max = 1;
  for (int c = 0; c < 3; ++c) if (p.st_strips[c]) { bsh_min = std::min(bsh_min, p.fh[c] / 2); bshb_max = std::max(bshb_max, p.fh[c] / 4); }
  int grp = 1;
  auto lds_of = [&](int g) {
    int nll = 4;
    while (nll < g * bshb_max) nll *= 2;
    return (size_t)g * imgA + (size_t)(g + 1) * imgB + (b_last ? 0 : (size_t)nll * 64 * (store16 ? 4 : 8));
  };
  while (grp * 2 * bsh_min <= 8 && lds_of(grp * 2) <= 20 * 1024) grp *= 2;
  static const int force_grp = vc2_tune_int("VC2HIP_PAIR_GROUP", 0);
  if (force_grp > 0) grp = force_grp;
  int nll = 4;
  while (nll < grp * bshb_max) nll *= 2;
  pp.grp_a = grp;
  pp.sz_a = (int)(imgA / elem);
  pp.sz_b = (int)(imgB / elem);
  pp.img_b = (int)(grp * imgA);
  pp.ring_ll = (int)(grp * imgA + (grp + 1) * imgB);
  pp.n_ll = nll;
  const size_t lds = inverse ? 16 : lds_of(grp);
  if (lds > 48 * 1024) return 0;
  int cols = 0;
  for (int c = 0; c < 3; ++c) if (p.st_strips[c]) cols += p.st_strips[c] * n_pictures;
  const int slots = pair_slots(kernel, edge, inverse, store16, lds);
  if (slots <= 0) return 0;
  const int runin = -3 * t.sd + 3 * t.offl + 8;
  int nseg = 0;
  long long best = -1;
  for (int g = 1; g <= p.ys; ++g) {
    bool ok = true;
// ... 39 lines not shown
```

vc2-reference_amd/csrc/vc2hip_internal.h:

```cpp
#pragma once

#include <hip/hip_runtime.h>
#include <hip/hip_ext.h>
#include <stddef.h>
#include <stdint.h>

#include "../../include/vc2hip.h"

#define VC2_MAX_DEPTH 7
#define VC2_MAX_BANDS (3 * VC2_MAX_DEPTH + 1)

enum : unsigned {
  VC2_DEVERR_QINDEX = 1u << 0,
  VC2_DEVERR_SCALAR = 1u << 1,
  VC2_DEVERR_CBR_TOOBIG = 1u << 2,
  VC2_DEVERR_CBR_LEN = 1u << 3,
  VC2_DEVERR_CODE32 = 1u << 4,
  VC2_DEVERR_STREAM = 1u << 5,
  VC2_DEVERR_LD_TOOBIG = 1u << 6,
  VC2_DEVERR_HANDOFF = 1u << 7,
  VC2_DEVERR_CAP = 1u << 8,
  VC2_DEVERR_SYNTAX = 1u << 9,
};
#define VC2_ERRBLK_SYNTAX_AT 8
// ... 96 lines not shown
};
__device__ __forceinline__ int vc2_norm(int x, int n) { return (x + (1 << (n - 1))) >> n; }

__host__ __device__ __forceinline__ long long vc2_raw_pic_offset(long long stride, int field_step, int field_shift, int pic) {
  return (long long)(pic >> field_shift) * stride + (long long)(pic & field_shift) * field_step;
}
__host__ __device__ __forceinline__ long long vc2_raw_pic_offset(const LevelParams &p, int comp, int pic) {
  return vc2_raw_pic_offset(p.plane_stride[comp], p.field_step[comp], p.field_shift, pic);
}

struct RawPlane {
  long long stride;
  int pitch, field_step, field_shift;
  int le, lsb;
};
#define VC2_PERM_RD_BE 0x02030001u
#define VC2_PERM_RD_LE 0x03020100u
#define VC2_PERM_WR_BE 0x04050001u
#define VC2_PERM_WR_LE 0x05040100u
__device__ __forceinline__ unsigned vc2_load_word(const uint8_t *q, int wb, int le) {
  unsigned u = 0;
  if (le) for (int b = 0; b < wb; ++b) u |= (unsigned)q[b] << (8 * b);
  else for (int b = 0; b < wb; ++b) u = (u << 8) | q[b];
  return u;
}
__device__ __forceinline__ void vc2_store_word(uint8_t *q, unsigned u, int wb, int le) {
  for (int b = 0; b < wb; ++b) q[b] = (uint8_t)(u >> (8 * (le ? b : wb - 1 - b)));
}

struct PairParams {
  LevelParams a, b;
  int spl[3];
  int img_b;
  int grp_a;
  int sz_a, sz_b;
  int ring_ll, n_ll;
  int ss_a[3], ss_b[3];
  int piece_a[3], piece_b[3];
};

#include <stdlib.h>
#ifdef VC2HIP_ABLATE
static inline int vc2_tune_int(const char *name, int def) { const char *e = getenv(name); return e ? atoi(e) : def; }
#else
static inline int vc2_tune_int(const char *, int def) { return def; }
#endif

#ifdef VC2HIP_ABLATE
#define VC2_SKIP(p, bit) (((p).debug_skip & (bit)) != 0)
#else
#define VC2_SKIP(p, bit) false
#endif

struct PackParams {
  const void *store;
  const int32_t *store_wide;
  int store16;
  long long store_stride;
  const int32_t *qidx;
  int n_slices, slice_coefs;
  int comp_n[3], comp_off[3], comp_n0[3];
  int depth;
  int prefix, scalar;
  int qmatrix[VC2_MAX_BANDS];
  uint8_t *slots;
  int slot_bytes;
  uint32_t *sizes;
  int tile_slices;
  const int32_t *cbr_bytes;
  const uint32_t *cbr_offsets;
  uint8_t *payload;
  long long payload_stride;
  unsigned *err;
  int quantise;
  int big_lut;
  float inv_scalar;
  union {
    unsigned char band_lut[768];
    unsigned lane16[200];
  };
  int debug_skip;
  unsigned long long *lookback;
  long long lookback_stride;
  unsigned long long *lens;
};

constexpr int VC2_BP_MAX = 3;
struct BandPlanes {
  int levels;
  int bytes8;
  int from[3];
  long long base[3][VC2_BP_MAX];
  int ow[3][VC2_BP_MAX], np[3][VC2_BP_MAX];
  int lbsh[3][VC2_BP_MAX], lbsw[3][VC2_BP_MAX];
};

struct HeadSplit {
  int n[3];
  long long base[3];
};

struct UnpackParams {
  const uint8_t *payload;
  long long payload_stride;
  const unsigned long long *lens;
  const uint32_t *offsets;
  void *store;
  int32_t *store_wide;
  int store16;
  long long store_stride;
  int32_t *qidx;
  int n_slices, slice_coefs;
  int comp_n[3], comp_off[3];
  int prefix, scalar;
  unsigned *err;
  BandPlanes bp;
  HeadSplit hs;
  int xs;
  unsigned long long *stats;
  int debug_skip;
};

struct CbrParams {
  const void *store;
  const int32_t *store_wide;
  int store16;
  long long store_stride;
  int32_t *qidx;
  const int32_t *slice_bytes;
  int n_slices, slice_coefs;
  int comp_n[3], comp_off[3], comp_n0[3];
  int scalar;
  int n_bands;
  int qmatrix[VC2_MAX_BANDS];
  unsigned *err;
  int only_marked;
  int general_only;
  float inv_scalar;
  int qm_min;
  union {
    unsigned char band_lut[768];
    unsigned lane8[72];
  };
};
#define VC2_CBR_MARK 0x7FFFFFFF

#define VC2_CAP_Q_TOP 115
#define VC2_CAP_ROW 32
#define VC2_CAP_R2 16
#define VC2_CAP_BASE 24
#define VC2_CAP_COUNT 25
#define VC2_CAP_ELSE 26
#define VC2_CAP_NOFIT (1ull << 40)
struct CapParams {
  CbrParams s;
  unsigned long long *table;
  unsigned long long cap;
  int prefix, floor;
  int round;
};

struct Launcher;
void vc2_prof_pair(Launcher &L, hipEvent_t *a, hipEvent_t *b);
#define VC2_LAUNCH(L, kernel, grid, block, lds, s, ...)                                        \
  do {                                                                                         \
    hipEvent_t vc2_ev_a_, vc2_ev_b_;                                                           \
    vc2_prof_pair(L, &vc2_ev_a_, &vc2_ev_b_);                                                  \
    hipExtLaunchKernelGGL(kernel, grid, block, lds, s, vc2_ev_a_, vc2_ev_b_, 0, __VA_ARGS__);  \
  } while (0)

void vc2_allow_lds(const void *kernel, size_t bytes);

void vc2_upload_tables(const QuantTables &t, hipStream_t s);
int vc2_launch_forward_level(Launcher &L, int kernel, bool first, const LevelParams &p, int n_pictures,
                             hipStream_t s);
int vc2_launch_inverse_level(Launcher &L, int kernel, bool final_level, const LevelParams &p,
                             int n_pictures, hipStream_t s);
size_t vc2_level_lds_bytes(int kernel, const LevelParams &p);

void vc2_launch_pack(Launcher &L, const PackParams &p, int n_pictures, hipStream_t s);
int vc2_pack_slices_per_tile(const PackParams &p);
bool vc2_pack_one_pass_default(const PackParams &p);
void vc2_launch_scan_sizes(Launcher &L, const uint32_t *sizes, uint32_t *offsets,
                           unsigned long long *totals, int n_slices, int n_pictures, hipStream_t s);
void vc2_launch_compact(Launcher &L, const uint8_t *slots, int slot_bytes, const uint32_t *sizes,
                        const uint32_t *offsets, uint8_t *payload, long long payload_stride,
                        int n_slices, int n_pictures, hipStream_t s);
void vc2_launch_cbr(Launcher &L, const CbrParams &p, int n_pictures, hipStream_t s);
void vc2_launch_cap(Launcher &L, const CapParams &p, int n_pictures, hipStream_t s);
void vc2_launch_unpack(Launcher &L, const UnpackParams &p, int n_pictures, hipStream_t s);
void vc2_launch_cbr_index(Launcher &L, const uint8_t *payload, long long stride, const unsigned long long *lens, const int32_t *budget,
                          const uint32_t *cbr_offs, unsigned long long total, uint32_t *offsets, int n_slices, int prefix, int scalar,
                          int n_pictures, unsigned *bad, hipStream_t s);
void vc2_launch_slice_index(Launcher &L, const uint8_t *payload, long long payload_stride,
                            const unsigned long long *lens, uint32_t *offsets, int n_slices,
                            int prefix, int scalar, int n_pictures, unsigned *err, hipStream_t s,
                            void *workspace, size_t workspace_bytes, const unsigned *skip = nullptr);
size_t vc2_slice_index_workspace(int n_pictures, size_t max_payload, int prefix, int scalar);

void vc2_launch_plane_to_store(Launcher &L, const int32_t *plane, int ph, int pw, int depth, int ys,
                               int xs, int32_t *store, int slice_coefs, int coef_off, hipStream_t s);
void vc2_launch_store_to_plane(Launcher &L, const int32_t *store, int slice_coefs, int coef_off,
                               int32_t *plane, int ph, int pw, int depth, int ys, int xs,
                               const int32_t *qidx, const int *qmatrix, int mode ,
                               unsigned *err, hipStream_t s);
void vc2_launch_quantise_store(Launcher &L, int32_t *store, int n_slices, int slice_coefs, int comp_n,
                               int comp_off, int n0, const int32_t *qidx, const int *qmatrix,
                               unsigned *err, hipStream_t s);
struct LdLl3Params {
  const int32_t *store;
  long long store_stride;
  int slice_coefs, coef_off[3], llh[3], llw[3], ys, xs;
  const int32_t *qidx;
  int qm0;
  int32_t *ll_plane[3];
  long long ll_stride[3];
  unsigned *err;
};
bool vc2_launch_ld_ll3(Launcher &L, const LdLl3Params &p, int n_pictures, hipStream_t s);
void vc2_launch_ld_ll(Launcher &L, const int32_t *store, long long store_stride, int slice_coefs,
                      int coef_off, int n0, int llh, int llw, int ys, int xs, const int32_t *qidx,
                      int qm0, int32_t *ll_plane, long long ll_stride, int n_pictures, unsigned *err,
                      hipStream_t s);
struct LdUnpackParams {
  const uint8_t *payload;
  long long payload_stride;
  const int32_t *slice_bytes;
  const uint32_t *offsets;
  int32_t *store;
  long long store_stride;
  int32_t *qidx;
  int n_slices, slice_coefs;
  int comp_n[3], comp_off[3];
  unsigned *err;
  const unsigned long long *lens;
// ... 154 lines not shown
```

vc2-reference_amd/csrc/vc2hip_pack16.h:

```cpp
#pragma once

#ifdef VC2HIP_ABLATE
__device__ unsigned g_p16_stats[8];
#define P16_STAT(k, cond) do { if (VC2_SKIP(p, 8) && __any(cond) && lane == 0) atomicAdd(&g_p16_stats[k], 1u); } while (0)
#else
#define P16_STAT(k, cond)
#endif
constexpr int P16_LUT_N = 256;
constexpr int P16_MAXQ = 126;
__device__ unsigned g_vlc_lut_s[P16_LUT_N];

static void fill_vlc_lut_s(unsigned *host) {
  for (int i = 0; i < P16_LUT_N; ++i) {
    const int t = i < 128 ? i : i - 256;
    const unsigned m = (unsigned)(t < 0 ? -t : t);
    unsigned code = 1, nb = 1;
    if (m) {
      const unsigned v = m + 1;
      int k = 31;
      while (!((v >> k) & 1u)) --k;
      code = 0;
      for (int b = k - 1; b >= 0; --b) code = (code << 2) | ((v >> b) & 1u);
      code = (((code << 1) | 1u) << 1) | (t < 0 ? 1u : 0u);
      nb = 2 * (unsigned)k + 2;
// ... 50 lines not shown
      }
      start += size;
    }
    if (start != n) return false;
    if (head < 0) head = n;
    if (head & 7) return false;
    lane16[64 + c] = (unsigned)head;
    lane16[67 + c] = (unsigned)((n - head) / 16);
    body_lanes += (n - head) / 16;
  }
  return body_lanes >= 40;
}

__device__ __forceinline__ void p16_group(const uint4 w, const float f, const unsigned *lut, unsigned long long &G, int &L,
                                          int &last, float &maxf) {
  const unsigned ww[4] = {w.x, w.y, w.z, w.w};
  unsigned pr[4];
  int pl[4];
  int S = 0;
  last = 0;
#pragma unroll
  for (int d = 0; d < 4; ++d) {
    const float f0 = (float)(int)(short)(ww[d] & 0xFFFFu), f1 = (float)((int)ww[d] >> 16);
    maxf = fmaxf(maxf, fmaxf(__builtin_fabsf(f0), __builtin_fabsf(f1)));
    const int t0 = (int)(f0 * f), t1 = (int)(f1 * f);
    const unsigned e0 = lut[t0 & 0xFF], e1 = lut[t1 & 0xFF];
    const int l0 = (int)(e0 >> 24), l1 = (int)(e1 >> 24);
    S += l0;
    const int c0 = S & (int)(signed char)(e0 >> 16);
    S += l1;
    const int c1 = S & (int)(signed char)(e1 >> 16);
    last = max(last, max(c0, c1));
    pr[d] = ((e0 & 0xFFFFu) << l1) | (e1 & 0xFFFFu);
    pl[d] = l0 + l1;
  }
  const unsigned long long q0 = ((unsigned long long)pr[0] << pl[1]) | pr[1], q1 = ((unsigned long long)pr[2] << pl[3]) | pr[3];
  G = (q0 << (pl[2] + pl[3])) | q1;
  L = S;
}


__device__ __forceinline__ void p16_put(unsigned *img, int pos, unsigned long long G, int n, int keep) {
  const unsigned long long v = (G >> (n - keep)) << ((64 - keep) & 63);
  const unsigned hi = (unsigned)(v >> 32), lo = (unsigned)v;
  unsigned *at = img + (pos >> 5);
  const unsigned bo = (unsigned)pos;
  atomicOr(at, __builtin_amdgcn_alignbit(0u, hi, bo));
  atomicOr(at + 1, __builtin_amdgcn_alignbit(hi, lo, bo));
  atomicOr(at + 2, __builtin_amdgcn_alignbit(lo, 0u, bo));
}

template <bool WRITE>
__device__ __forceinline__ int p16_general(const int16_t *src, const int32_t *srcw, int n, int n0, int q, const int *qm, int lane,
                                        unsigned *img, int bit0, int region_bits, unsigned *err) {
  const int n0_shift = (n0 & (n0 - 1)) == 0 ? 31 - __clz(n0) : -1;
  int base = 0, count = 0;
#pragma unroll 1
  for (int r0 = 0; r0 < n; r0 += 64) {
    const int j = r0 + lane;
    int c = 0, nb = 0;
    if (j < n) {
      const int aq = max(q - qm[band_of_index_fast(j, n0, n0_shift)], 0);
      if (aq > 119) atomicOr(err, VC2_DEVERR_QINDEX);
      else c = quant_dev(St<int16_t>::load1(src + j, srcw + j), aq);
      nb = svlc_bits(c);
      if (nb > 32) { atomicOr(err, VC2_DEVERR_CODE32); c = 0; nb = 1; }
    }
    const int incl = wave_incl_scan(nb, lane), pos = base + incl - nb;
    if (WRITE) { if (nb && pos + nb <= region_bits) put_code(img, bit0 + pos, svlc_code(c), nb); }
    else count = max(count, wave_max(c != 0 ? pos + nb : 0));
    base += __builtin_amdgcn_readlane(incl, 63);
  }
  return count;
}

constexpr int P16_SLOTS = 0, P16_CBR = 1, P16_LOOKBACK = 2;
#ifndef VC2_P16LB_WPE
#define VC2_P16LB_WPE 8
#endif
template <int MODE>
__global__ __launch_bounds__((MODE == 2 ? 64 * P16LB_WAVES : 256), (MODE == 2 ? VC2_P16LB_WPE : 1)) void k_hq_pack16(const PackParams p) {
  constexpr bool CBR = MODE == P16_CBR, LB = MODE == P16_LOOKBACK;
  extern __shared__ unsigned lds_u[];
  constexpr int NW = MODE == 2 ? P16LB_WAVES : 4;
  __shared__ int s_tot[NW];
  const int lane = threadIdx.x & 63, wave = __builtin_amdgcn_readfirstlane(threadIdx.x >> 6);
  const int pic = LB ? blockIdx.x : blockIdx.y, tile = LB ? blockIdx.y : blockIdx.x;
  const int slice = tile * NW + wave;
  const bool active = slice < p.n_slices;
  const int img_q = ((p.prefix + 4 + 3 * 255 * p.scalar + 3) / 4 + 2 + 3) / 4;
  unsigned *lut = lds_u;
  uint4 *qt = (uint4 *)(lds_u + P16_LUT_N);
  unsigned *img = lds_u + P16_LUT_N + 4 * 128 + wave * img_q * 4;
  unsigned lut_e = 0x04000002u;
  uint4 qt_e = make_uint4(0u, 0u, 0x40000000u, 0u);
  if (!VC2_SKIP(p, 4)) {
    lut_e = g_vlc_lut_s[threadIdx.x & (P16_LUT_N - 1)];
    qt_e = g_p16_qt[threadIdx.x & 127];
  }
  const unsigned lt = p.lane16[lane];
  const int comp = lane < 32 ? 0 : (lane < 48 ? 1 : 2), cl = lane - (lane < 32 ? 0 : (lane < 48 ? 32 : 48));
  const int head_n = (int)(comp == 0 ? p.lane16[64] : (comp == 1 ? p.lane16[65] : p.lane16[66]));
  const int body_n = (int)(comp == 0 ? p.lane16[67] : (comp == 1 ? p.lane16[68] : p.lane16[69]));
  const int coff = comp == 0 ? p.comp_off[0] : (comp == 1 ? p.comp_off[1] : p.comp_off[2]);
  const bool has_body = cl < body_n, has_head = cl < head_n;
  const size_t rec_at = (size_t)pic * p.store_stride + (size_t)(active ? slice : 0) * p.slice_coefs;
  const int16_t *rec = (const int16_t *)p.store + rec_at;
  uint4 w0 = make_uint4(0u, 0u, 0u, 0u), w1 = w0;
  int hv = 0;
  if (active && has_body) { const int16_t *b = rec + coff + head_n + 16 * cl; w0 = *(const uint4 *)b; w1 = *(const uint4 *)(b + 8); }
  if (active && has_head) hv = rec[coff + cl];
  const int32_t *hwide = p.store_wide + rec_at + coff + cl;
  const int q = p.qidx[(size_t)pic * p.n_slices + (active ? slice : 0)];
  if (threadIdx.x < P16_LUT_N) lut[threadIdx.x] = lut_e;
  if (threadIdx.x < 128) qt[threadIdx.x] = qt_e;
  for (int i = lane; i < img_q; i += 64) ((uint4 *)img)[i] = make_uint4(0u, 0u, 0u, 0u);
  __syncthreads();
  if (!active) {
    if constexpr (LB) {
      if (lane == 0) s_tot[wave] = 0;
      __syncthreads();
      __syncthreads();
    }
    return;
  }

  const int aqb = max(q - (int)(lt & 0xFFu), 0), aqh = max(q - (int)((lt >> 8) & 0xFFu), 0);
  if ((has_body && aqb > 119) || (has_head && aqh > 119)) atomicOr(p.err, VC2_DEVERR_QINDEX);
  const float fb = __uint_as_float(qt[min(aqb, 120)].w);
  const uint4 qh = qt[min(aqh, 120)];

  unsigned long long G0, G1;
  int L0, L1, last0, last1;
  float maxf = 0.f;
  p16_group(w0, fb, lut, G0, L0, last0, maxf);
  p16_group(w1, fb, lut, G1, L1, last1, maxf);
  int body_bits = L0 + L1, body_last = last1 ? L0 + last1 : last0;
  bool slow = maxf >= 32768.f  || maxf * fb >= (float)(P16_MAXQ + 1) || max(L0, L1) > 63;
  if (!has_body) { body_bits = 0; body_last = 0; slow = false; }
  unsigned hcode = 0;
  int hbits = 0;
  bool hnz = false;
  if (has_head) {
    if (hv == VC2_ST_SENTINEL) hv = *hwide;
    const int t = quant_core(hv, (int)qh.z, qh.x, (int)qh.y);
    slow |= (unsigned)(t + 65534) > 2u * 65534u;
    hcode = svlc_code(t);
    hbits = svlc_bits(t);
    hnz = t != 0;
  }

  const int cbr_total = CBR ? p.cbr_bytes[slice] : 0;
  bool bad_cbr = false;
  int bytes[3];
  auto comp_len = [&](int count) -> int {
    int len = (int)((float)(((count + 7) >> 3) + p.scalar - 1) * p.inv_scalar);
    if (len > 255) { atomicOr(p.err, VC2_DEVERR_SCALAR); len = 255; }
    return len * p.scalar;
  };
  auto cbr_v = [&](int need) -> int {
    if (!CBR) return need;
    const int vb = cbr_total - 4 - bytes[0] - bytes[1];
    if (vb < need) { if (lane == 0) atomicOr(p.err, VC2_DEVERR_CBR_TOOBIG); bad_cbr = true; return need; }
    if (vb / p.scalar > 255) { if (lane == 0) atomicOr(p.err, VC2_DEVERR_CBR_LEN); bad_cbr = true; return need; }
    return vb;
  };

  P16_STAT(0, true); P16_STAT(1, has_body && maxf >= 32768.f); P16_STAT(2, has_body && maxf * fb >= (float)(P16_MAXQ + 1));
  P16_STAT(3, has_body && max(L0, L1) > 63); P16_STAT(4, slow);
  unsigned long long lb_first = 0;
  bool lb_have = false;
  unsigned *wimg = img;
  int wb = 0;
  const int leader = LB ? (tile == (p.n_slices + NW - 1) / NW - 1 ? 0 : (tile & (NW - 1))) : 0;
  auto lb_publish = [&](int total_bytes) {
    if (lane == 0) s_tot[wave] = total_bytes;
    __syncthreads();
    wimg = lds_u + P16_LUT_N + 4 * 128;
    {
      int b = 0;
#pragma unroll
      for (int w2 = 0; w2 < NW - 1; ++w2) b += wave > w2 ? s_tot[w2] : 0;
      wb = __builtin_amdgcn_readfirstlane(b);
    }
    if (wave == leader && tile > 0) {
      unsigned long long *st = p.lookback + (size_t)pic * p.lookback_stride + 1;
      int agg = 0;
#pragma unroll
      for (int w2 = 0; w2 < NW; ++w2) agg += s_tot[w2];
      if (lane == 0) __hip_atomic_store(&st[tile], (1ull << 62) | (unsigned long long)agg, __ATOMIC_RELAXED, __HIP_MEMORY_SCOPE_AGENT);
      const int t = tile - 1 - lane;
      lb_first = t >= 0 ? __hip_atomic_load(&st[t], __ATOMIC_RELAXED, __HIP_MEMORY_SCOPE_AGENT) : (2ull << 62);
      lb_have = true;
    }
  };
  const bool slow_any = __any(slow);
  if (__builtin_expect(slow_any, 0)) {
    const int32_t *recw = p.store_wide + rec_at;
    if constexpr (LB) {
#pragma unroll 1
      for (int cc = 0; cc < 3; ++cc)
        bytes[cc] = comp_len(p16_general<false>(rec + p.comp_off[cc], recw + p.comp_off[cc], p.comp_n[cc], p.comp_n0[cc], q, p.qmatrix, lane, nullptr, 0, 0, p.err));
      lb_publish(p.prefix + 4 + bytes[0] + bytes[1] + bytes[2]);
    }
    int base = p.prefix + 1;
    for (int cc = 0; cc < 3; ++cc) {
      const int16_t *src = rec + p.comp_off[cc];
      const int32_t *srcw = recw + p.comp_off[cc];
      if constexpr (!LB) {
        const int count = p16_general<false>(src, srcw, p.comp_n[cc], p.comp_n0[cc], q, p.qmatrix, lane, nullptr, 0, 0, p.err);
        bytes[cc] = comp_len(count);
        if (cc == 2) bytes[2] = cbr_v(bytes[2]);
      }
      p16_general<true>(src, srcw, p.comp_n[cc], p.comp_n0[cc], q, p.qmatrix, lane, wimg, 8 * (wb + base + 1), 8 * bytes[cc], p.err);
      if (lane == 0) put_byte(wimg, wb + base, (unsigned)(bytes[cc] / p.scalar));
      base += 1 + bytes[cc];
    }
    if (lane == 0) put_byte(wimg, wb + p.prefix, (unsigned)q & 0xFFu);
  } else {
    const int pk = (hbits << 16) | body_bits;
    int s = pk;
    s += dpp0<0x111, 0xf>(s);
    s += dpp0<0x112, 0xf>(s);
    s += dpp0<0x114, 0xf>(s);
    s += dpp0<0x118, 0xf>(s);
    s += dpp0<0x142, 0x2>(s);
    const int tot_y = __builtin_amdgcn_readlane(s, 31), tot_u = __builtin_amdgcn_readlane(s, 47), tot_v = __builtin_amdgcn_readlane(s, 63);
    const int tot = comp == 0 ? tot_y : (comp == 1 ? tot_u : tot_v);
    const int excl = s - pk;
    const int hpos = excl >> 16, bpos = (tot >> 16) + (excl & 0xFFFF);
    const int endpos = body_last ? bpos + body_last : (hnz ? hpos + hbits : 0);
    const unsigned long long nzb = __ballot(body_last != 0), nzh = __ballot(hnz);
    auto count_of = [&](unsigned b, unsigned h, int lane0) -> int {
      const unsigned m = b ? b : h;
      return m ? __builtin_amdgcn_readlane(endpos, lane0 + 31 - __builtin_clz(m)) : 0;
    };
    const int cnt_y = count_of((unsigned)nzb, (unsigned)nzh, 0);
    const int cnt_u = count_of((unsigned)(nzb >> 32) & 0xFFFFu, (unsigned)(nzh >> 32) & 0xFFFFu, 32);
    const int cnt_v = count_of((unsigned)(nzb >> 48), (unsigned)(nzh >> 48), 48);
    const int len = comp_len(lane == 0 ? cnt_y : (lane == 1 ? cnt_u : cnt_v));
    bytes[0] = __builtin_amdgcn_readlane(len, 0);
    bytes[1] = __builtin_amdgcn_readlane(len, 1);
    bytes[2] = cbr_v(__builtin_amdgcn_readlane(len, 2));
    if constexpr (LB) lb_publish(p.prefix + 4 + bytes[0] + bytes[1] + bytes[2]);
    const int at_u = p.prefix + 2 + bytes[0], at_v = at_u + 1 + bytes[1];
    const int bit0 = 8 * (wb + (comp == 0 ? p.prefix + 1 : (comp == 1 ? at_u : at_v)) + 1);
    const int room = 8 * (comp == 0 ? bytes[0] : (comp == 1 ? bytes[1] : bytes[2]));
    if (hbits && hpos + hbits <= room) {
      const unsigned v = hcode << (32 - hbits);
      unsigned *at = wimg + ((bit0 + hpos) >> 5);
      const unsigned bo = (unsigned)(bit0 + hpos);
      atomicOr(at, __builtin_amdgcn_alignbit(0u, v, bo));
      atomicOr(at + 1, __builtin_amdgcn_alignbit(v, 0u, bo));
    }
    if (has_body) {
      const int keep = min(max(room - bpos, 0), body_bits), k0 = min(keep, L0);
      p16_put(wimg, bit0 + bpos, G0, L0, k0);
      p16_put(wimg, bit0 + bpos + L0, G1, L1, keep - k0);
    }
    if (lane < 4) {
      const int at = lane == 0 ? p.prefix : (lane == 1 ? p.prefix + 1 : (lane == 2 ? at_u : at_v));
      const int lb = lane == 1 ? bytes[0] : (lane == 2 ? bytes[1] : bytes[2]);
      const unsigned val = lane == 0 ? ((unsigned)q & 0xFFu) : (unsigned)((float)lb * p.inv_scalar);
      put_byte(wimg, wb + at, val);
    }
  }
  const int total = p.prefix + 4 + bytes[0] + bytes[1] + bytes[2];
// ... 266 lines not shown
```

vc2-reference_amd/csrc/vc2hip_slices.hip:

```cpp
#include <stdlib.h>

#include <algorithm>
#include <atomic>
#include <mutex>

#include "vc2hip_internal.h"
#include "vc2hip_store.h"

void vc2_prof_begin(Launcher &L, const char *name, hipStream_t s);
void vc2_prof_end(Launcher &L, hipStream_t s);

__constant__ QuantTables c_qs;
void vc2_upload_p16_tables(const QuantTables &t, hipStream_t s);
void vc2_upload_tables_slices(const QuantTables &t, hipStream_t s) {
  (void)hipMemcpyToSymbolAsync(HIP_SYMBOL(c_qs), &t, sizeof t, 0, hipMemcpyHostToDevice, s);
  vc2_upload_p16_tables(t, s);
}

__device__ __forceinline__ int quant_core(int v, int qf, unsigned mg, int sh) {
  const unsigned mag = v < 0 ? 0u - (unsigned)v : (unsigned)v;
  const int a = (int)(mag << 2);
  const unsigned t = __umulhi(mg, (unsigned)a);
  int q = (int)((t + (((unsigned)a - t) >> 1)) >> sh);
  const bool slow = !(qf > 1 && a >= 0);
// ... 678 lines not shown

struct __attribute__((aligned(4))) Dword4 { unsigned x, y, z, w; };
#include "vc2hip_pack16.h"

size_t vc2_pack_lds_bytes(int prefix, int scalar);
static size_t pack_lds(int prefix, int scalar, int slices_per_wave, bool big_lut = false, int waves = 4, bool gimg = false) {
  const size_t img_words = gimg ? 0 : ((size_t)prefix + 4 + 3 * 255 * (size_t)scalar + 3) / 4 + 2;
  return waves * slices_per_wave * img_words * 4 + VLC_LUT_N * 4 + 768 + waves * (size_t)slices_per_wave * 32 * 16 + (big_lut ? 4096 : 0);
}
int vc2_pack_image_mode(int prefix, int scalar) {
  if (pack_lds(prefix, scalar, 1) <= 144 * 1024) return 0;
  if (pack_lds(prefix, scalar, 1, false, 2) <= 144 * 1024) return 2;
  if (pack_lds(prefix, scalar, 1, false, 1) <= 144 * 1024) return 1;
  return -1;
}
size_t vc2_pack_lds_bytes(int prefix, int scalar) { return pack_lds(prefix, scalar, 1); }
static int pack_lanes(const PackParams &p) {
  int W = 64;
  const bool same_c = p.comp_n[1] == p.comp_n[2];
  static const int force_w = vc2_tune_int("VC2HIP_PACK_LANES", 0);
  if (!p.lookback && same_c && force_w != 64) {
    const int bands = 3 * p.depth + 1;
    if (p.comp_n[0] <= 128 && p.comp_n[1] <= 64 && bands <= 16 && pack_lds(p.prefix, p.scalar, 4) <= 144 * 1024) W = 16;
    else if (p.comp_n[0] <= 256 && p.comp_n[1] <= 128 && bands <= 32 && pack_lds(p.prefix, p.scalar, 2) <= 144 * 1024) W = 32;
  }
  return W;
}
int vc2_pack_slices_per_tile(const PackParams &p) {
  if (vc2_pack_image_mode(p.prefix, p.scalar) != 0) return 0;
  const int W = pack_lanes(p);
  return W == 64 ? 0 : 4 * (64 / W);
}
#ifdef VC2HIP_ABLATE
static void p16_print_stats(hipStream_t s) {
  static const bool on = getenv("VC2HIP_P16_STATS") != nullptr;
  if (!on) return;
  unsigned h[8], z[8] = {0, 0, 0, 0, 0, 0, 0, 0};
  (void)hipStreamSynchronize(s);
  (void)hipMemcpyFromSymbol(h, HIP_SYMBOL(g_p16_stats), sizeof h);
  (void)hipMemcpyToSymbol(HIP_SYMBOL(g_p16_stats), z, sizeof z);
  fprintf(stderr, "pack16: wavefronts %u, store escape %u, quotient beyond the table %u, string beyond 63 bits %u, general path %u\n", h[0], h[1], h[2], h[3], h[4]);
}
#else
static void p16_print_stats(hipStream_t) {}
#endif
bool vc2_pack_one_pass_default(const PackParams &p0) {
  static const int use16 = vc2_tune_int("VC2HIP_PACK16", 1);
  if (!use16 || p0.cbr_bytes || vc2_pack_image_mode(p0.prefix, p0.scalar) != 0) return false;
  PackParams p = p0;
  static unsigned long long dummy;
  p.lookback = &dummy;
  p.tile_slices = 0;
  return pack16_plan(p, p.lane16);
}
void vc2_launch_pack(Launcher &L, const PackParams &p0, int n_pictures, hipStream_t s) {
  PackParams p = p0;
#ifdef VC2HIP_ABLATE
  { const char *e = getenv("VC2HIP_DEBUG_PACK"); p.debug_skip = (e ? atoi(e) : 0) | (getenv("VC2HIP_P16_STATS") ? 8 : 0); }
#endif
  p.inv_scalar = 1.0f / (float)p.scalar;
  if ((double)p.inv_scalar < 1.0 / (double)p.scalar) p.inv_scalar = nextafterf(p.inv_scalar, INFINITY);
  static const int use16 = vc2_tune_int("VC2HIP_PACK16", 1);
  if (use16 && vc2_pack_image_mode(p.prefix, p.scalar) == 0 && pack16_plan(p, p.lane16)) {
    const size_t lds = pack16_lds(p.prefix, p.scalar);
    const dim3 grid((p.n_slices + 3) / 4, n_pictures);
    vc2_prof_begin(L, "hq_pack", s);
    if (p.cbr_bytes) {
      vc2_allow_lds((const void *)k_hq_pack16<P16_CBR>, 144 * 1024);
      VC2_LAUNCH(L, k_hq_pack16<P16_CBR>, grid, dim3(256), lds, s, p);
    } else if (p.lookback) {
      vc2_allow_lds((const void *)k_hq_pack16<P16_LOOKBACK>, 144 * 1024);
      VC2_LAUNCH(L, k_hq_pack16<P16_LOOKBACK>, dim3(n_pictures, (p.n_slices + P16LB_WAVES - 1) / P16LB_WAVES), dim3(64 * P16LB_WAVES),
                 pack16_lds(p.prefix, p.scalar, P16LB_WAVES), s, p);
    } else {
      vc2_allow_lds((const void *)k_hq_pack16<P16_SLOTS>, 144 * 1024);
      VC2_LAUNCH(L, k_hq_pack16<P16_SLOTS>, grid, dim3(256), lds, s, p);
    }
    vc2_prof_end(L, s);
    p16_print_stats(s);
    return;
  }
  if (use16 && pack16w_lds(p.prefix, p.scalar) <= 64 * 1024 && pack16w_plan(p, p.lane16)) {
    const size_t lds = pack16w_lds(p.prefix, p.scalar);
    const dim3 grid(p.n_slices, n_pictures);
    vc2_prof_begin(L, "hq_pack", s);
    if (p.cbr_bytes) {
      vc2_allow_lds((const void *)k_hq_pack16w<true>, 64 * 1024);
      VC2_LAUNCH(L, k_hq_pack16w<true>, grid, dim3(192), lds, s, p);
    } else {
      vc2_allow_lds((const void *)k_hq_pack16w<false>, 64 * 1024);
      VC2_LAUNCH(L, k_hq_pack16w<false>, grid, dim3(192), lds, s, p);
    }
    vc2_prof_end(L, s);
    p16_print_stats(s);
    return;
  }
  fill_band_lut(p.band_lut, p.comp_n, p.comp_n0);
  const int W = pack_lanes(p);
  const bool same_c = p.comp_n[1] == p.comp_n[2];
  const int S = 64 / W;
  const bool one_round = p.comp_n[0] <= 512 && p.comp_n[1] <= 256 && same_c;
  p.big_lut = W == 64 && !one_round && same_c && p.comp_n[0] <= 2048 && p.comp_n[1] <= 2048 && 3 * p.depth + 1 <= 32 &&
              pack_lds(p.prefix, p.scalar, 1, true) <= 144 * 1024;
  const int mode = vc2_pack_image_mode(p.prefix, p.scalar);
  if (mode != 0) {
    const int waves = mode < 0 ? 4 : mode;
// ... 2780 lines not shown
```

vc2-reference_amd/vc2hip_py.py:

```python
import ctypes as C
import math
import os

import numpy as np

HERE = os.path.dirname(os.path.abspath(__file__))
LIB_PATH = os.environ.get("VC2HIP_LIB") or os.path.join(HERE, "libvc2hip.so")

i32p = np.ctypeslib.ndpointer(dtype=np.int32, flags="C_CONTIGUOUS")
u8p = np.ctypeslib.ndpointer(dtype=np.uint8, flags="C_CONTIGUOUS")

FLAGS = {"STORE32": 0x001, "NO_STREAM": 0x002, "NO_PAIR": 0x004, "NO_BANDPLANES": 0x008, "NO_HEADS": 0x010, "NO_CBR_INDEX": 0x020,
         "GENERIC_DWT": 0x040, "SINGLE_PASS_VBR": 0x080, "CBR_GENERAL": 0x100, "LD_DIAGONALS": 0x200,
         "PLANES8_ALWAYS": 0x400, "PLANES8_NEVER": 0x800, "TWO_PASS_VBR": 0x1000, "CAP_GENERAL": 0x2000}

KERNELS = {"DD97": 0, "LeGall": 1, "DD137": 2, "Haar0": 3, "Haar1": 4, "Fidelity": 5, "Daub97": 6}
CF = {"444": 0, "422": 1, "420": 2}
MODES = {"HQ_ConstQ": 0, "HQ_CBR": 1, "LD": 2, "HQ_Capped": 3}


class Geom(C.Structure):
    _fields_ = [("luma_h", C.c_int), ("luma_w", C.c_int), ("chroma_h", C.c_int),
                ("chroma_w", C.c_int), ("depth", C.c_int), ("y_slices", C.c_int),
                ("x_slices", C.c_int)]


class PictureFormat(C.Structure):
    _fields_ = [("width", C.c_int), ("height", C.c_int), ("chroma_format", C.c_int),
                ("bit_depth", C.c_int), ("word_bytes", C.c_int), ("chroma_bit_depth", C.c_int)]


class CodingParams(C.Structure):
    _fields_ = [("kernel", C.c_int), ("depth", C.c_int), ("y_slices", C.c_int),
                ("x_slices", C.c_int), ("mode", C.c_int), ("q_index", C.c_int),
                ("compressed_bytes", C.c_int), ("prefix", C.c_int), ("scalar", C.c_int)]


class DwtLaunch(C.Structure):
    _fields_ = [("inverse", C.c_int), ("level", C.c_int), ("levels", C.c_int), ("family", C.c_int), ("edge", C.c_int),
                ("store_bits", C.c_int), ("segments", C.c_int), ("tail", C.c_int), ("small_gather", C.c_int),
                ("pictures", C.c_int), ("band_planes", C.c_int)]


class StreamParams(C.Structure):
    _fields_ = [("major_version", C.c_int), ("first_picture_number", C.c_uint32), ("prev_parse_offset", C.c_uint32),
                ("end_of_sequence", C.c_int)]


class SampleLayout(C.Structure):
    _fields_ = [("little_endian", C.c_int), ("lsb_justified", C.c_int), ("pitch", C.c_size_t * 3),
                ("plane_offset", C.c_size_t * 3), ("picture_stride", C.c_size_t)]


class PackedFormat(C.Structure):
    _fields_ = [("packing", C.c_int), ("little_endian", C.c_int), ("lsb_justified", C.c_int), ("pitch", C.c_size_t * 2),
                ("plane_offset", C.c_size_t * 2), ("picture_stride", C.c_size_t)]


PACKING = {"none": 0, "v210": 1, "semiplanar": 2}
DWT_FAMILIES = ("tile", "fast", "stream", "pair", "plane")


class Vc2HipError(RuntimeError):
    def __init__(self, code, msg):
        super().__init__(msg)
        self.code = code


EXPORTS = [
    "vc2hip_create", "vc2hip_create_with_flags", "vc2hip_create_on_stream", "vc2hip_create_on_stream_with_flags", "vc2hip_destroy",
    "vc2hip_last_error",
    "vc2hip_error_string", "vc2hip_sync", "vc2hip_padded_size", "vc2hip_slice_size_is_valid",
    "vc2hip_quant_matrix", "vc2hip_slice_bytes", "vc2hip_dwt_forward", "vc2hip_dwt_inverse",
    "vc2hip_quantise_np", "vc2hip_dequantise_np", "vc2hip_dequantise_ld", "vc2hip_hq_pack",
    "vc2hip_hq_unpack", "vc2hip_ld_unpack", "vc2hip_cbr_qindices", "vc2hip_quantise_ld", "vc2hip_ld_pack",
    "vc2hip_ld_qindices", "vc2hip_encode_picture_ld", "vc2hip_set_streams", "vc2hip_raw_picture_bytes",
    "vc2hip_max_payload_bytes", "vc2hip_encode_picture_hq", "vc2hip_decode_picture_hq",
    "vc2hip_decode_picture_ld", "vc2hip_encode_batch_dev", "vc2hip_decode_batch_dev",
    "vc2hip_profile_enable", "vc2hip_profile_only", "vc2hip_profile_count", "vc2hip_profile_get", "vc2hip_profile_reset",
    "vc2hip_host_alloc", "vc2hip_host_free", "vc2hip_encode_picture_begin", "vc2hip_encode_picture_end",
    "vc2hip_decode_picture_begin", "vc2hip_decode_picture_end", "vc2hip_band_plane_bits", "vc2hip_dwt_launches",
    "vc2hip_picture_header", "vc2hip_stream_write_dev", "vc2hip_stream_read_dev",
    "vc2hip_encode_fields_batch_dev", "vc2hip_decode_fields_batch_dev", "vc2hip_decode_reduced_batch_dev",
    "vc2hip_encode_recon_batch_dev", "vc2hip_stream_write_fragments_dev",
    "vc2hip_set_sample_layout", "vc2hip_layout_picture_bytes",
    "vc2hip_set_packed_format", "vc2hip_packed_picture_bytes",
]


def load_library():
    if not os.path.exists(LIB_PATH):
        raise RuntimeError(f"{LIB_PATH} is missing: run `python -c 'import __graft_entry__ as g; g.build()'` "
                           "(there is no CPU fallback)")
    if os.environ.get("VC2HIP_NO_TORCH") != "1":
        try:
            import torch
        except Exception:
            pass
    lib = C.CDLL(LIB_PATH)
    vp = C.c_void_p
    lib.vc2hip_create.argtypes = [C.c_int, C.POINTER(vp)]
    lib.vc2hip_create_with_flags.argtypes = [C.c_int, C.c_uint, C.POINTER(vp)]
    lib.vc2hip_create_on_stream.argtypes = [C.c_int, vp, C.POINTER(vp)]
    lib.vc2hip_create_on_stream_with_flags.argtypes = [C.c_int, vp, C.c_uint, C.POINTER(vp)]
    lib.vc2hip_destroy.argtypes = [vp]
    lib.vc2hip_destroy.restype = None
    lib.vc2hip_last_error.argtypes = [vp]
    lib.vc2hip_last_error.restype = C.c_char_p
    lib.vc2hip_error_string.argtypes = [C.c_int]
    lib.vc2hip_error_string.restype = C.c_char_p
    lib.vc2hip_sync.argtypes = [vp]
    lib.vc2hip_set_streams.argtypes = [vp, C.c_int]
    lib.vc2hip_quant_matrix.argtypes = [C.c_int, C.c_int, i32p]
    lib.vc2hip_slice_bytes.argtypes = [C.c_int, C.c_int, C.c_int, C.c_int, i32p]
    lib.vc2hip_dwt_forward.argtypes = [vp, i32p, C.c_int, C.c_int, C.c_int, C.c_int, i32p]
    lib.vc2hip_dwt_inverse.argtypes = [vp, i32p, C.c_int, C.c_int, C.c_int, C.c_int, i32p, C.c_int, C.c_int]
    for f in (lib.vc2hip_quantise_np, lib.vc2hip_dequantise_np, lib.vc2hip_dequantise_ld, lib.vc2hip_quantise_ld):
        f.argtypes = [vp, i32p, C.c_int, C.c_int, C.c_int, i32p, C.c_int, C.c_int, i32p, i32p]
    lib.vc2hip_hq_pack.argtypes = [vp, i32p, i32p, i32p, C.POINTER(Geom), i32p, C.c_int, C.c_int,
                                   vp, u8p, C.c_size_t, C.POINTER(C.c_size_t)]
    lib.vc2hip_hq_unpack.argtypes = [vp, u8p, C.c_size_t, C.POINTER(Geom), C.c_int, C.c_int, i32p,
                                     i32p, i32p, i32p, C.POINTER(C.c_size_t)]
    lib.vc2hip_ld_unpack.argtypes = [vp, u8p, C.c_size_t, C.POINTER(Geom), i32p, i32p, i32p, i32p,
                                     i32p, C.POINTER(C.c_size_t)]
    lib.vc2hip_cbr_qindices.argtypes = [vp, i32p, i32p, i32p, C.POINTER(Geom), i32p, i32p, C.c_int, i32p]
    lib.vc2hip_ld_qindices.argtypes = [vp, i32p, i32p, i32p, C.POINTER(Geom), i32p, i32p, i32p]
    lib.vc2hip_ld_pack.argtypes = [vp, i32p, i32p, i32p, C.POINTER(Geom), i32p, i32p, u8p, C.c_size_t,
                                   C.POINTER(C.c_size_t)]
    lib.vc2hip_raw_picture_bytes.argtypes = [C.POINTER(PictureFormat)]
    lib.vc2hip_raw_picture_bytes.restype = C.c_size_t
    lib.vc2hip_max_payload_bytes.argtypes = [C.POINTER(PictureFormat), C.POINTER(CodingParams)]
    lib.vc2hip_max_payload_bytes.restype = C.c_size_t
    for f in (lib.vc2hip_encode_picture_hq, lib.vc2hip_encode_picture_ld):
        f.argtypes = [vp, u8p, C.POINTER(PictureFormat), C.POINTER(CodingParams), u8p, C.c_size_t,
                      C.POINTER(C.c_size_t), vp]
    for f in (lib.vc2hip_decode_picture_hq, lib.vc2hip_decode_picture_ld):
        f.argtypes = [vp, u8p, C.c_size_t, C.POINTER(PictureFormat), C.POINTER(CodingParams), u8p]
    lib.vc2hip_encode_batch_dev.argtypes = [vp, vp, C.c_int, C.POINTER(PictureFormat),
                                            C.POINTER(CodingParams), vp, C.c_size_t, vp]
    lib.vc2hip_decode_batch_dev.argtypes = [vp, vp, C.c_size_t, vp, C.c_int, C.POINTER(PictureFormat),
                                            C.POINTER(CodingParams), vp]
    lib.vc2hip_encode_fields_batch_dev.argtypes = [vp, vp, C.c_int, C.POINTER(PictureFormat), C.c_int,
                                                   C.POINTER(CodingParams), vp, C.c_size_t, vp]
    lib.vc2hip_decode_fields_batch_dev.argtypes = [vp, vp, C.c_size_t, vp, C.c_int, C.POINTER(PictureFormat), C.c_int,
                                                   C.POINTER(CodingParams), vp]
    lib.vc2hip_decode_reduced_batch_dev.argtypes = [vp, vp, C.c_size_t, vp, C.c_int, C.POINTER(PictureFormat),
                                                    C.POINTER(CodingParams), C.c_int, vp]
    lib.vc2hip_encode_recon_batch_dev.argtypes = [vp, vp, C.c_int, C.POINTER(PictureFormat), C.POINTER(CodingParams),
                                                  vp, C.c_size_t, vp, vp, vp, vp]
    lib.vc2hip_set_sample_layout.argtypes = [vp, C.POINTER(SampleLayout)]
    lib.vc2hip_layout_picture_bytes.argtypes = [C.POINTER(PictureFormat), C.POINTER(SampleLayout)]
    lib.vc2hip_layout_picture_bytes.restype = C.c_size_t
    lib.vc2hip_set_packed_format.argtypes = [vp, C.POINTER(PackedFormat)]
    lib.vc2hip_packed_picture_bytes.argtypes = [C.POINTER(PictureFormat), C.POINTER(PackedFormat)]
    lib.vc2hip_packed_picture_bytes.restype = C.c_size_t
    lib.vc2hip_picture_header.argtypes = [C.POINTER(CodingParams), C.c_int, C.c_uint32, u8p, C.c_size_t,
                                          C.POINTER(C.c_size_t)]
    lib.vc2hip_stream_write_dev.argtypes = [vp, vp, C.c_size_t, vp, C.c_int, C.POINTER(CodingParams), C.POINTER(StreamParams),
                                            vp, C.c_size_t, vp]
    lib.vc2hip_stream_write_fragments_dev.argtypes = [vp, vp, C.c_size_t, vp, C.c_int, C.POINTER(CodingParams),
                                                      C.POINTER(StreamParams), C.c_int, vp, C.c_size_t, vp, vp, C.c_size_t, vp]
    lib.vc2hip_stream_read_dev.argtypes = [vp, vp, C.c_size_t, C.c_int, C.POINTER(CodingParams), C.POINTER(StreamParams),
                                           vp, C.c_size_t, vp, vp, vp]
    lib.vc2hip_profile_enable.argtypes = [vp, C.c_int]
    lib.vc2hip_profile_only.argtypes = [vp, C.c_char_p]
    lib.vc2hip_profile_count.argtypes = [vp]
    lib.vc2hip_profile_get.argtypes = [vp, C.c_int, C.POINTER(C.c_char_p), C.POINTER(C.c_int),
                                       C.POINTER(C.c_double)]
    lib.vc2hip_profile_reset.argtypes = [vp]
    lib.vc2hip_band_plane_bits.argtypes = [vp]
    lib.vc2hip_dwt_launches.argtypes = [vp, C.POINTER(DwtLaunch), C.c_int]
    lib.vc2hip_host_alloc.argtypes = [C.c_size_t]
    lib.vc2hip_host_alloc.restype = vp
    lib.vc2hip_host_free.argtypes = [vp]
    lib.vc2hip_host_free.restype = None
    lib.vc2hip_encode_picture_begin.argtypes = [vp, vp, C.POINTER(PictureFormat), C.POINTER(CodingParams), vp, C.c_size_t, vp,
                                                C.POINTER(C.c_int)]
    lib.vc2hip_encode_picture_end.argtypes = [vp, C.c_int, C.POINTER(C.c_size_t)]
    lib.vc2hip_decode_picture_begin.argtypes = [vp, vp, C.c_size_t, C.POINTER(PictureFormat), C.POINTER(CodingParams), vp,
                                                C.POINTER(C.c_int)]
    lib.vc2hip_decode_picture_end.argtypes = [vp, C.c_int]
    return lib


def picture_format(width, height, cf, bits, word_bytes=2, chroma_bits=0):
    return PictureFormat(width, height, CF[cf], bits, word_bytes, chroma_bits)


def reduced_format(fmt, drop_levels):
    return PictureFormat(fmt.width >> drop_levels, fmt.height >> drop_levels, fmt.chroma_format, fmt.bit_depth, fmt.word_bytes,
                         fmt.chroma_bit_depth)


def sample_layout(little_endian=False, lsb_justified=False, pitch=(0, 0, 0), plane_offset=(0, 0, 0), picture_stride=0):
    return SampleLayout(int(little_endian), int(lsb_justified), (C.c_size_t * 3)(*pitch), (C.c_size_t * 3)(*plane_offset),
                        picture_stride)


def layout_picture_bytes(lib, fmt, layout=None):
    return lib.vc2hip_layout_picture_bytes(C.byref(fmt), C.byref(layout) if layout is not None else None)


def packed_format(packing, little_endian=False, lsb_justified=False, pitch=(0, 0), plane_offset=(0, 0), picture_stride=0):
    return PackedFormat(PACKING.get(packing, packing), int(little_endian), int(lsb_justified), (C.c_size_t * 2)(*pitch),
                        (C.c_size_t * 2)(*plane_offset), picture_stride)


def v210_pitch(width, align=128):
    return ((width + 5) // 6 * 16 + align - 1) // align * align


def packed_picture_bytes(lib, fmt, pf):
    return lib.vc2hip_packed_picture_bytes(C.byref(fmt), C.byref(pf) if pf is not None else None)


def torch_planes(y, u, v):
    ts = (y, u, v)
    if any(t.dim() != 3 for t in ts):
        raise ValueError("torch_planes: every plane must have shape (n, rows, cols)")
    if len({t.dtype for t in ts}) != 1 or len({t.device for t in ts}) != 1:
        raise ValueError("torch_planes: the planes must share dtype and device")
    wb = y.element_size()
    if y.is_floating_point() or y.is_complex() or wb not in (1, 2):
# ... 306 lines not shown
        outs = [self.lib.vc2hip_host_alloc(rb + 64) for _ in range(n_slots)]
        res, open_ = [], []
        try:
            def finish():
                slot, ticket = open_.pop(0)
                self._chk(self.lib.vc2hip_decode_picture_end(self.h, ticket))
                res.append(C.string_at(outs[slot], rb))
            for k, pay in enumerate(payloads):
                if len(open_) == n_slots:
                    finish()
                slot = k % n_slots
                C.memmove(ins[slot], pay, len(pay))
                t = C.c_int()
                self._chk(self.lib.vc2hip_decode_picture_begin(self.h, ins[slot], len(pay), C.byref(fmt), C.byref(cp), outs[slot],
                                                               C.byref(t)))
                open_.append((slot, t.value))
            while open_:
                finish()
        finally:
            for p in ins + outs:
                self.lib.vc2hip_host_free(p)
        return res

    def set_sample_layout(self, layout=None):
        self._chk(self.lib.vc2hip_set_sample_layout(self.h, C.byref(layout) if layout is not None else None))

    def layout_picture_bytes(self, fmt, layout=None):
        return layout_picture_bytes(self.lib, fmt, layout)

    def set_packed_format(self, pf=None):
        self._chk(self.lib.vc2hip_set_packed_format(self.h, C.byref(pf) if pf is not None else None))

    def packed_picture_bytes(self, fmt, pf):
        return packed_picture_bytes(self.lib, fmt, pf)

    def set_streams(self, k):
        self._chk(self.lib.vc2hip_set_streams(self.h, k))

    def sync(self):
        self._chk(self.lib.vc2hip_sync(self.h))

    def profile_enable(self, on=True):
        self.lib.vc2hip_profile_enable(self.h, 1 if on else 0)

    def profile_only(self, name=None):
        self.lib.vc2hip_profile_only(self.h, name.encode() if name else None)

    def profile_reset(self):
        self.lib.vc2hip_profile_reset(self.h)

    def band_plane_bits(self):
        return int(self.lib.vc2hip_band_plane_bits(self.h))

    def dwt_launches(self):
        n = self.lib.vc2hip_dwt_launches(self.h, None, 0)
        self._chk(min(n, 0))
        buf = (DwtLaunch * max(n, 1))()
        n = self.lib.vc2hip_dwt_launches(self.h, buf, n)
        out = []
        for r in buf[:n]:
            d = {name: getattr(r, name) for name, _ in DwtLaunch._fields_}
            d["family"] = DWT_FAMILIES[d["family"]]
            out.append(d)
        return out

    def profile(self):
        out = {}
        for i in range(self.lib.vc2hip_profile_count(self.h)):
            name = C.c_char_p()
            n = C.c_int()
            ms = C.c_double()
            self.lib.vc2hip_profile_get(self.h, i, C.byref(name), C.byref(n), C.byref(ms))
            out[name.value.decode()] = (n.value, ms.value)
        return out
```

Baseline: 123,700 Mpixels/s.

## Write forward DWT coarse-level coefficients into contiguous head planes for the pack16 coder

In the HQ ConstQ encode path the forward two-level pair launch for the deepest levels now writes the low-resolution 'head' coefficients into separate contiguous per-component regions placed after the slice store. The 16-bit packer reads heads from those regions, with index remapping on the slow path, instead of gathering them per slice. The layout plan is computed once, cached by a geometry key, and validated against the pair launch and the pack16 plan. This is meant to make head loads in the pack kernel and writes in the DWT more coalesced, at the cost of a larger wide-store buffer and extra planning logic.

```diff
diff --git a/include/vc2hip.h b/include/vc2hip.h
--- a/include/vc2hip.h
+++ b/include/vc2hip.h
@@ -51,6 +51,7 @@
 #define VC2HIP_FLAG_PLANES8_NEVER   0x800u
 #define VC2HIP_FLAG_TWO_PASS_VBR    0x1000u
 #define VC2HIP_FLAG_CAP_GENERAL     0x2000u
+#define VC2HIP_FLAG_NO_FWD_HEADS    0x4000u
 int vc2hip_create_with_flags(int device, unsigned flags, vc2hip_ctx **out);
 int vc2hip_create_on_stream(int device, void *hip_stream, vc2hip_ctx **out);
 int vc2hip_create_on_stream_with_flags(int device, void *hip_stream, unsigned flags, vc2hip_ctx **out);
@@ -212,6 +213,8 @@
 
 int vc2hip_band_plane_bits(const vc2hip_ctx *ctx);
 
+int vc2hip_forward_heads(const vc2hip_ctx *ctx);
+
 #define VC2HIP_DWT_TILE   0
 #define VC2HIP_DWT_FAST   1
 #define VC2HIP_DWT_STREAM 2
diff --git a/vc2-reference_amd/csrc/vc2hip_api.hip b/vc2-reference_amd/csrc/vc2hip_api.hip
--- a/vc2-reference_amd/csrc/vc2hip_api.hip
+++ b/vc2-reference_amd/csrc/vc2hip_api.hip
@@ -162,6 +162,11 @@
   double stat_samples = 0;
   int ld_batch = 1;
   bool allow_heads = true;
+  bool allow_fwd_heads = true;
+  int last_fwd_heads = 0;
+  int fwd_heads_key[40] = {-1};
+  HeadSplit fwd_heads_plan = {};
+  long long fwd_heads_stride = 0;
   bool allow_cbr_index = true;
   bool allow_stream = true;
   bool allow_pair = true;
@@ -336,6 +341,7 @@
     static const struct { const char *name; unsigned flag; } env[] = {
       {"VC2HIP_STORE32", VC2HIP_FLAG_STORE32}, {"VC2HIP_NO_STREAM", VC2HIP_FLAG_NO_STREAM}, {"VC2HIP_NO_PAIR", VC2HIP_FLAG_NO_PAIR},
       {"VC2HIP_NO_BANDPLANES", VC2HIP_FLAG_NO_BANDPLANES}, {"VC2HIP_NO_HEADS", VC2HIP_FLAG_NO_HEADS},
+      {"VC2HIP_NO_FWD_HEADS", VC2HIP_FLAG_NO_FWD_HEADS},
       {"VC2HIP_NO_CBR_INDEX", VC2HIP_FLAG_NO_CBR_INDEX}, {"VC2HIP_GENERIC_DWT", VC2HIP_FLAG_GENERIC_DWT},
       {"VC2HIP_SINGLE_PASS_VBR", VC2HIP_FLAG_SINGLE_PASS_VBR}, {"VC2HIP_TWO_PASS_VBR", VC2HIP_FLAG_TWO_PASS_VBR}, {"VC2HIP_CBR_GENERAL", VC2HIP_FLAG_CBR_GENERAL}, {"VC2HIP_CAP_GENERAL", VC2HIP_FLAG_CAP_GENERAL},
       {"VC2HIP_PLANES8_ALWAYS", VC2HIP_FLAG_PLANES8_ALWAYS}, {"VC2HIP_PLANES8_NEVER", VC2HIP_FLAG_PLANES8_NEVER}};
@@ -351,6 +357,7 @@
   c->allow_planes = !(flags & VC2HIP_FLAG_NO_BANDPLANES);
   c->planes8_mode = (flags & VC2HIP_FLAG_PLANES8_NEVER) ? 2 : (flags & VC2HIP_FLAG_PLANES8_ALWAYS) ? 1 : 0;
   c->allow_heads = !(flags & VC2HIP_FLAG_NO_HEADS);
+  c->allow_fwd_heads = !(flags & VC2HIP_FLAG_NO_FWD_HEADS);
   c->allow_cbr_index = !(flags & VC2HIP_FLAG_NO_CBR_INDEX);
   c->two_pass_vbr = !(flags & VC2HIP_FLAG_SINGLE_PASS_VBR);
   c->force_two_pass_vbr = (flags & VC2HIP_FLAG_TWO_PASS_VBR) != 0;
@@ -897,11 +904,15 @@
 
 static int run_forward(vc2hip_ctx *c, const Geom &g, int kernel, int n, const void *const src[3],
                        const RawPlane src_l[3], bool src_raw, const vc2hip_picture_format *f,
-                       void *store, const LLPlanes &ll, bool s16 = false, int32_t *store_wide = nullptr) {
+                       void *store, const LLPlanes &ll, bool s16 = false, int32_t *store_wide = nullptr,
+                       const HeadSplit *hs = nullptr, int head_level = 1 << 30, long long store_stride = 0, bool *heads_pair = nullptr) {
+  if (heads_pair) *heads_pair = false;
   auto level_params = [&](LevelParams &p, int level) {
     memset(&p, 0, sizeof p);
     fill_level(p, g, level, kernel, nullptr);
-    p.store = store; p.store_stride = (long long)g.ys * g.xs * g.slice_coefs;
+    if (hs && level >= head_level)
+      for (int k = 0; k < 3; ++k) if (g.c[k].ph) { p.rec_stride[k] = hs->n[k]; p.coef_off[k] = (int)hs->base[k]; }
+    p.store = store; p.store_stride = store_stride ? store_stride : (long long)g.ys * g.xs * g.slice_coefs;
     p.store_wide = store_wide;
     p.err = c->d_err;
     p.ll_to_store = (level == g.depth - 1);
@@ -939,7 +950,13 @@
       pp.a.debug_skip = c->debug_skip;
       level_params(pp.b, level + 1);
       const size_t lds = vc2_pair_applicable(pp, kernel, first, false, s16, n);
+      if (lds && heads_pair) {
+        if (level == head_level && !first && level + 2 == g.depth) *heads_pair = true;
+        ++level;
+        continue;
+      }
       if (lds) {
+        if (hs && level + 1 >= head_level && (level != head_level || first)) return set_err(c, VC2HIP_EINVAL, "internal: forward heads without their two-level launch");
         int rc = vc2_launch_forward_pair(c->L, kernel, first, pp, n, s16, lds, c->stream);
         if (rc) return set_err(c, rc, "invalid wavelet kernel");
         record_dwt(c, false, level, 2, VC2HIP_DWT_PAIR, first, s16, pp.a.st_segmax, 0, false, n);
@@ -947,6 +964,8 @@
         continue;
       }
     }
+    if (heads_pair) continue;
+    if (hs && level >= head_level) return set_err(c, VC2HIP_EINVAL, "internal: forward heads without their two-level launch");
     LevelParams pf = p;
     pf.debug_skip = c->debug_skip;
     if (!c->force_generic && c->allow_stream) {
@@ -1158,31 +1177,58 @@
   for (int c = 0; c < 3; ++c) { n[c] = g.c[c].sh * g.c[c].sw; off[c] = g.c[c].coef_off; n0[c] = g.c[c].n0 ? g.c[c].n0 : 1; }
 }
 
-static int run_pack(vc2hip_ctx *c, const Geom &g, int n, const void *store, const int32_t *d_qidx,
-                    const int32_t *qm, bool quantise, int prefix, int scalar, const int32_t *d_cbr_bytes,
-                    const uint32_t *d_cbr_offs, uint64_t cbr_total, uint8_t *d_payload, long long stride,
-                    unsigned long long *d_lens, bool s16 = false, const int32_t *store_wide = nullptr) {
-  const int ns = g.ys * g.xs;
-  PackParams p;
+struct PackRoute {
+  bool gimg;
+  bool one_pass;
+  int spt;
+};
+static void fill_pack(vc2hip_ctx *c, PackParams &p, const Geom &g, const void *store, const int32_t *d_qidx, const int32_t *qm, bool quantise,
+                      int prefix, int scalar, bool s16, const int32_t *store_wide) {
   memset(&p, 0, sizeof p);
-  p.store = store; p.store_stride = (long long)ns * g.slice_coefs;
+  p.store = store; p.store_stride = (long long)g.ys * g.xs * g.slice_coefs;
   p.store16 = s16; p.store_wide = store_wide;
-  p.qidx = d_qidx; p.n_slices = ns; p.slice_coefs = g.slice_coefs;
+  p.qidx = d_qidx; p.n_slices = g.ys * g.xs; p.slice_coefs = g.slice_coefs;
   fill_comp_arrays(g, p.comp_n, p.comp_off, p.comp_n0);
   p.depth = g.depth; p.prefix = prefix; p.scalar = scalar;
   for (int b = 0; b < 3 * g.depth + 1; ++b) p.qmatrix[b] = qm ? qm[b] : 0;
   p.err = c->d_err; p.quantise = quantise;
+}
+static PackRoute pack_route(const vc2hip_ctx *c, const PackParams &p, int n, bool cbr) {
+  PackRoute r;
+  r.gimg = vc2_pack_image_mode(p.prefix, p.scalar) < 0;
+  r.one_pass = !r.gimg && !cbr &&
+               (!c->two_pass_vbr || (!c->force_two_pass_vbr && n >= VC2_ONE_PASS_MIN_PICTURES && vc2_pack_one_pass_default(p)));
+  r.spt = (r.gimg || cbr || r.one_pass) ? 0 : vc2_pack_slices_per_tile(p);
+  return r;
+}
+
+static int run_pack(vc2hip_ctx *c, const Geom &g, int n, const void *store, const int32_t *d_qidx,
+                    const int32_t *qm, bool quantise, int prefix, int scalar, const int32_t *d_cbr_bytes,
+                    const uint32_t *d_cbr_offs, uint64_t cbr_total, uint8_t *d_payload, long long stride,
+                    unsigned long long *d_lens, bool s16 = false, const int32_t *store_wide = nullptr,
+                    const HeadSplit *hs = nullptr, long long store_stride = 0) {
+  const int ns = g.ys * g.xs;
+  PackParams p;
+  fill_pack(c, p, g, store, d_qidx, qm, quantise, prefix, scalar, s16, store_wide);
   p.payload = d_payload; p.payload_stride = stride;
-  const bool gimg = vc2_pack_image_mode(prefix, scalar) < 0;
+  const PackRoute route = pack_route(c, p, n, d_cbr_bytes != nullptr);
+  const bool gimg = route.gimg;
+  if (hs) {
+    p.hs = *hs; p.store_stride = store_stride;
+    PackParams q = p;
+    static unsigned long long dummy;
+    if (route.one_pass) q.lookback = &dummy; else q.tile_slices = route.spt;
+    int head[3];
+    if (d_cbr_bytes || !vc2_pack16_heads(q, head) || head[0] != hs->n[0] || head[1] != hs->n[1] || head[2] != hs->n[2])
+      return set_err(c, VC2HIP_EINVAL, "internal: forward heads without the coder that reads them");
+  }
   if (d_cbr_bytes && !gimg) {
     p.cbr_bytes = d_cbr_bytes; p.cbr_offsets = d_cbr_offs;
     vc2_launch_pack(c->L, p, n, c->stream);
     vc2_launch_fill_u64(c->L, d_lens, cbr_total, (size_t)n, c->stream);
     return VC2HIP_OK;
   }
-  const bool one_pass = !gimg && !d_cbr_bytes &&
-                        (!c->two_pass_vbr || (!c->force_two_pass_vbr && n >= VC2_ONE_PASS_MIN_PICTURES && vc2_pack_one_pass_default(p)));
-  if (one_pass) {
+  if (route.one_pass) {
     const long long lb_stride = (long long)((ns + 3) / 4) + 8;
     unsigned long long *lb;
     NEED(c, B_SIZES, (size_t)n * lb_stride * 8, lb);
@@ -1194,14 +1240,13 @@
   }
   const int slot = (int)((max_slice_bytes(prefix, scalar) + (gimg ? 8 : 0) + 15) & ~(size_t)15);
   uint8_t *slots; uint32_t *sizes, *offs;
-  const int spt_room = (gimg || d_cbr_bytes) ? 0 : vc2_pack_slices_per_tile(p);
-  const size_t slot_count = spt_room ? (size_t)((ns + spt_room - 1) / spt_room) * spt_room : (size_t)ns;
+  const int spt = route.spt;
+  const size_t slot_count = spt ? (size_t)((ns + spt - 1) / spt) * spt : (size_t)ns;
   NEED(c, B_SLOTS, (size_t)n * slot_count * slot + 32, slots);
   NEED(c, B_SIZES, (size_t)n * ns * 4, sizes);
   NEED(c, B_OFFS, (size_t)n * ns * 4, offs);
   p.slots = slots; p.slot_bytes = slot; p.sizes = sizes;
   if (d_cbr_bytes) { p.cbr_bytes = d_cbr_bytes; p.cbr_offsets = d_cbr_offs; }
-  const int spt = (gimg || d_cbr_bytes) ? 0 : vc2_pack_slices_per_tile(p);
   p.tile_slices = spt;
   vc2_launch_pack(c->L, p, n, c->stream);
   if (spt) {
@@ -1905,6 +1950,55 @@
   return encode_batch_common(c, d_raw, 1, 1, n, f, cp, d_payload, payload_stride, d_lens, &ro);
 }
 
+static bool plan_forward_heads(vc2hip_ctx *c, const Geom &g, const vc2hip_coding_params *cp, int n, const vc2hip_picture_format *f,
+                               const int32_t *qm, const void *const src[3], const RawPlane ss[3], HeadSplit &hs, long long &sstride) {
+  int key[40];
+  memset(key, 0, sizeof key);
+  int at = 0;
+  for (int k = 0; k < 3; ++k) { const CompGeom &cg = g.c[k]; key[at++] = cg.h; key[at++] = cg.w; key[at++] = cg.ph; key[at++] = cg.pw; key[at++] = cg.sh; key[at++] = cg.sw; key[at++] = ss[k].pitch; }
+  key[at++] = g.depth; key[at++] = g.ys; key[at++] = g.xs; key[at++] = g.slice_coefs; key[at++] = cp->kernel; key[at++] = cp->prefix; key[at++] = cp->scalar;
+  key[at++] = n; key[at++] = f->word_bytes; key[at++] = 1;
+  if (!memcmp(key, c->fwd_heads_key, sizeof key)) { hs = c->fwd_heads_plan; sstride = c->fwd_heads_stride; return hs.n[0] != 0; }
+  memset(&hs, 0, sizeof hs);
+  const int ns = g.ys * g.xs, ls = g.depth - 2;
+  sstride = (long long)ns * g.slice_coefs;
+  auto decide = [&]() -> bool {
+    if (ls < 1 || c->force_generic || !c->allow_stream || !c->allow_pair) return false;
+    PackParams p;
+    fill_pack(c, p, g, nullptr, nullptr, qm, true, cp->prefix, cp->scalar, true, nullptr);
+    const PackRoute route = pack_route(c, p, n, false);
+    static unsigned long long dummy;
+    if (route.one_pass) p.lookback = &dummy; else p.tile_slices = route.spt;
+    int head[3];
+    if (!vc2_pack16_heads(p, head)) return false;
+    HeadSplit h;
+    memset(&h, 0, sizeof h);
+    long long end = sstride;
+    for (int k = 0; k < 3; ++k) {
+      if (!g.c[k].ph) return false;
+      const int hn = (g.c[k].sh >> ls) * (g.c[k].sw >> ls);
+      if (hn != head[k] || hn < 8 || (hn & 7)) return false;
+      h.n[k] = hn;
+      h.base[k] = end;
+      end += ((long long)ns * hn + 7) & ~7ll;
+    }
+    if (end >= (1ll << 31)) return false;
+    bool pair = false;
+    LLPlanes none;
+    memset(&none, 0, sizeof none);
+    (void)run_forward(c, g, cp->kernel, n, src, ss, true, f, nullptr, none, true, nullptr, &h, ls, end, &pair);
+    if (!pair) return false;
+    hs = h;
+    sstride = end;
+    return true;
+  };
+  const bool on = decide();
+  memcpy(c->fwd_heads_key, key, sizeof key);
+  c->fwd_heads_plan = hs;
+  c->fwd_heads_stride = sstride;
+  return on;
+}
+
 static int encode_batch_common(vc2hip_ctx *c, const void *d_raw, int fields, int top_first, int n, const vc2hip_picture_format *f,
                                const vc2hip_coding_params *cp, void *d_payload, size_t payload_stride, uint64_t *d_lens,
                                const ReconOut *ro) {
@@ -1927,16 +2021,6 @@
   int32_t qm[VC2_MAX_BANDS];
   if ((rc = vc2hip_quant_matrix(cp->kernel, cp->depth, qm))) return set_err(c, rc);
   const bool s16 = cp->mode != VC2HIP_LD && use_store16(c, g, cp->kernel);
-  int32_t *d_store, *d_ll, *d_q, *d_storew = nullptr, *d_llw = nullptr;
-  NEED(c, B_STORE, (size_t)n * ns * g.slice_coefs * 4, d_store);
-  NEED(c, B_LL0, ll_bytes(g, n) + 16, d_ll);
-  if (s16) {
-    NEED(c, B_STOREW, (size_t)n * ns * g.slice_coefs * 4, d_storew);
-    NEED(c, B_LLW, ll_bytes(g, n) + 16, d_llw);
-  }
-  NEED(c, B_QIDX, (size_t)n * ns * 4, d_q);
-  LLPlanes ll;
-  ll_layout(g, n, d_ll, s16 ? 2 : 4, d_llw, ll);
   const void *src[3]; RawPlane ss[3];
   RawView in;
   {
@@ -1944,11 +2028,30 @@
     fb.height = f->height * fields;
     if ((rc = raw_view(c, &fb, n / fields, d_raw, B_PKIN, in))) return rc;
   }
+  view_planes(in, f, fields, top_first, src, ss);
+  const bool plane_path = needs_plane_path(c, g, cp->kernel);
+  HeadSplit fhs;
+  memset(&fhs, 0, sizeof fhs);
+  long long sstride = (long long)ns * g.slice_coefs;
+  c->last_fwd_heads = 0;
+  if (s16 && c->allow_fwd_heads && cp->mode == VC2HIP_HQ_CONSTQ && !ro && d_payload && !plane_path &&
+      plan_forward_heads(c, g, cp, n, f, qm, src, ss, fhs, sstride))
+    c->last_fwd_heads = 1;
+  const HeadSplit *hs = c->last_fwd_heads ? &fhs : nullptr;
+  int32_t *d_store, *d_ll, *d_q, *d_storew = nullptr, *d_llw = nullptr;
+  NEED(c, B_STORE, (size_t)n * ns * g.slice_coefs * 4, d_store);
+  NEED(c, B_LL0, ll_bytes(g, n) + 16, d_ll);
+  if (s16) {
+    NEED(c, B_STOREW, (size_t)n * sstride * 4, d_storew);
+    NEED(c, B_LLW, ll_bytes(g, n) + 16, d_llw);
+  }
+  NEED(c, B_QIDX, (size_t)n * ns * 4, d_q);
+  LLPlanes ll;
+  ll_layout(g, n, d_ll, s16 ? 2 : 4, d_llw, ll);
   view_convert(c, in, false);
-  view_planes(in, f, fields, top_first, src, ss);
-  if (needs_plane_path(c, g, cp->kernel)) {
+  if (plane_path) {
     if ((rc = plane_forward(c, g, cp->kernel, n, src, ss, f, d_store))) return rc;
-  } else if ((rc = run_forward(c, g, cp->kernel, n, src, ss, true, f, d_store, ll, s16, d_storew))) return rc;
+  } else if ((rc = run_forward(c, g, cp->kernel, n, src, ss, true, f, d_store, ll, s16, d_storew, hs, hs ? g.depth - 2 : 1 << 30, sstride))) return rc;
   int32_t *d_cb = nullptr; uint32_t *d_co = nullptr; uint64_t total = 0;
   if (cp->mode == VC2HIP_LD) {
     const int key[5] = {g.ys, g.xs, cp->compressed_bytes, 1, -7};
@@ -2016,7 +2119,7 @@
     vc2_launch_fill_i32(c->L, d_q, cp->q_index, (size_t)n * ns, c->stream);
   }
   if (d_payload && (rc = run_pack(c, g, n, d_store, d_q, qm, true, cp->prefix, cp->scalar, d_cb, d_co, total, (uint8_t *)d_payload,
-                                  (long long)payload_stride, (unsigned long long *)d_lens, s16, d_storew))) return rc;
+                                  (long long)payload_stride, (unsigned long long *)d_lens, s16, d_storew, hs, sstride))) return rc;
   return ro ? run_recon(c, g, cp, n, f, qm, s16, d_store, d_storew, d_q, ll, in, *ro, d_cb, !d_payload, nullptr) : VC2HIP_OK;
 }
 
@@ -2323,6 +2426,7 @@
 }
 
 extern "C" int vc2hip_band_plane_bits(const vc2hip_ctx *c) { return c ? c->last_plane_bits : 0; }
+extern "C" int vc2hip_forward_heads(const vc2hip_ctx *c) { return c ? c->last_fwd_heads : 0; }
 
 namespace {
 struct HeaderBits {
diff --git a/vc2-reference_amd/csrc/vc2hip_dwt_pair.hip b/vc2-reference_amd/csrc/vc2hip_dwt_pair.hip
--- a/vc2-reference_amd/csrc/vc2hip_dwt_pair.hip
+++ b/vc2-reference_amd/csrc/vc2hip_dwt_pair.hip
@@ -73,7 +73,7 @@
   ST *imgA = (ST *)smem, *imgB = (ST *)(smem + pp.img_b);
   unsigned *ring_ll = (unsigned *)(smem + pp.ring_ll);
   const int szA = pp.sz_a, szB = pp.sz_b, grpA = pp.grp_a, nll = pp.n_ll;
-  const int xs = p.xs, slice_coefs = p.slice_coefs, st_prio = p.st_prio;
+  const int xs = p.xs, st_prio = p.st_prio;
 #ifdef VC2HIP_ABLATE
   const int dskip = p.debug_skip;
 #else
@@ -139,6 +139,7 @@
   const int b_last = pb.ll_to_store;
   const int run0A = p.coef_off[comp] + bnA, run0B = pb.coef_off[comp] + (b_last ? 0 : bnB);
   const int ssA = pp.ss_a[comp], ssB = pp.ss_b[comp];
+  const int rsA = p.rec_stride[comp], rsB = pb.rec_stride[comp];
   const int llps = p.st_llps[comp];
   const int si = spl == 1 ? (lane - sp.lo) >> llps : (lane - sp.lo) * spl;
   const int cl = spl == 1 ? (lane - sp.lo) & ((1 << llps) - 1) : 0;
@@ -152,11 +153,11 @@
     if constexpr (S_::narrow) llp_w = pb.ll_wide[comp] + (size_t)pic * pb.ll_stride[comp] + (size_t)chunk * 2;
   }
   const int baseA = si * ssA + cl * 4, baseB = si * ssB + cl * 2;
-  auto escapes = [&](int *v, auto NBc, auto NVc, int sv, int run0, int bn, int off_r, int clv) __attribute__((always_inline)) {
+  auto escapes = [&](int *v, auto NBc, auto NVc, int sv, int rs, int run0, int bn, int off_r, int clv) __attribute__((always_inline)) {
     constexpr int NB = decltype(NBc)::value, NV = decltype(NVc)::value, H = NV / 2;
     if constexpr (S_::narrow) {
-      int32_t *w0 = wide + mul24z(sv * xs + sp.sx0 + si, slice_coefs) + run0 + off_r + (spl == 1 ? clv : 0);
-      int32_t *w1 = spl == 1 ? w0 + H : w0 + slice_coefs;
+      int32_t *w0 = wide + mul24z(sv * xs + sp.sx0 + si, rs) + run0 + off_r + (spl == 1 ? clv : 0);
+      int32_t *w1 = spl == 1 ? w0 + H : w0 + rs;
 #pragma unroll
       for (int b = 0; b < NB; ++b, w0 += bn, w1 += bn)
 #pragma unroll
@@ -170,7 +171,7 @@
       int mx = v[0], mn = v[0];
 #pragma unroll
       for (int j = 1; j < 12; ++j) { mx = max(mx, v[j]); mn = min(mn, v[j]); }
-      if (__builtin_expect(mx > 32767 || mn < -32767, 0)) escapes(v, IC<3>(), IC<4>(), sv, run0A, bnA, r * bswA, cl * 4);
+      if (__builtin_expect(mx > 32767 || mn < -32767, 0)) escapes(v, IC<3>(), IC<4>(), sv, rsA, run0A, bnA, r * bswA, cl * 4);
     }
     ST *d = img + baseA + r * bswA;
 #pragma unroll
@@ -193,8 +194,8 @@
       for (int j = 3; j < 8; ++j) { mx = max(mx, v[j]); mn = min(mn, v[j]); }
       if (b_last) { mx = max(mx, max(v[0], v[1])); mn = min(mn, min(v[0], v[1])); }
       if (__builtin_expect(mx > 32767 || mn < -32767, 0)) {
-        if (b_last) escapes(v, IC<4>(), IC<2>(), sv, run0B, bnB, r * bswB, cl * 2);
-        else escapes(v + 2, IC<3>(), IC<2>(), sv, run0B, bnB, r * bswB, cl * 2);
+        if (b_last) escapes(v, IC<4>(), IC<2>(), sv, rsB, run0B, bnB, r * bswB, cl * 2);
+        else escapes(v + 2, IC<3>(), IC<2>(), sv, rsB, run0B, bnB, r * bswB, cl * 2);
       }
     }
     ST *d = img + baseB + r * bswB;
@@ -211,10 +212,10 @@
       d += bnB;
     }
   };
-  auto flush = [&](const ST *img, int ss, int run0, int run_n, int piece, int sv) __attribute__((always_inline)) {
+  auto flush = [&](const ST *img, int ss, int rs, int run0, int run_n, int piece, int sv) __attribute__((always_inline)) {
     const int epp = piece / (int)sizeof(ST), ppr = run_n / epp;
-    ST *rec0 = store + mul24z(sv * xs + sp.sx0, slice_coefs) + run0;
-    const bool nt = FIRST && VC2_PAIR_NT && piece == 16 && (((run0 | run_n | slice_coefs) * (int)sizeof(ST)) & 127) == 0;
+    ST *rec0 = store + mul24z(sv * xs + sp.sx0, rs) + run0;
+    const bool nt = FIRST && VC2_PAIR_NT && piece == 16 && (((run0 | run_n | rs) * (int)sizeof(ST)) & 127) == 0;
     if (ppr <= 64) {
       const int spt = 64 / ppr;
       int ls = (int)((float)lane * (1.0f / (float)ppr));
@@ -222,9 +223,9 @@
       ls += (ls + 1) * ppr <= lane ? 1 : 0;
       const int e = (lane - ls * ppr) * epp;
       const ST *src = img + ls * ss + e;
-      ST *dst = rec0 + mul24z(ls, slice_coefs) + e;
+      ST *dst = rec0 + mul24z(ls, rs) + e;
       const int dsrc = spt * ss;
-      const size_t ddst = mul24z(spt, slice_coefs);
+      const size_t ddst = mul24z(spt, rs);
 #pragma unroll 1
       for (int s2 = ls; s2 < sp.nsl; s2 += spt, src += dsrc, dst += ddst) {
         if (ls < spt) {
@@ -237,7 +238,7 @@
 #pragma unroll 1
       for (int s2 = 0; s2 < sp.nsl; ++s2) {
         const ST *src = img + s2 * ss;
-        ST *dst = rec0 + mul24z(s2, slice_coefs);
+        ST *dst = rec0 + mul24z(s2, rs);
 #pragma unroll 1
         for (int q = lane; q < ppr; q += 64) {
           if (piece == 16) { if (nt) st_nt(dst + q * epp, *(const uint4 *)(src + q * epp)); else *(uint4 *)(dst + q * epp) = *(const uint4 *)(src + q * epp); }
@@ -272,10 +273,10 @@
   auto burst = [&]() __attribute__((always_inline)) {
     wave_sync();
 #pragma unroll 1
-    for (; stA < dnA; ++stA) if (!(dskip & 256)) flush(imgA + ((stA - sv0) & (grpA - 1)) * szA, ssA, run0A, 3 * bnA, pieceA, stA);
+    for (; stA < dnA; ++stA) if (!(dskip & 256)) flush(imgA + ((stA - sv0) & (grpA - 1)) * szA, ssA, rsA, run0A, 3 * bnA, pieceA, stA);
 #pragma unroll 1
     for (; stB < dnB; ++stB) {
-      if (!(dskip & 64)) flush(imgB + slotBf * szB, ssB, run0B, (b_last ? 4 : 3) * bnB, pieceB, stB);
+      if (!(dskip & 64)) flush(imgB + slotBf * szB, ssB, rsB, run0B, (b_last ? 4 : 3) * bnB, pieceB, stB);
       slotBf = slotBf == grpA ? 0 : slotBf + 1;
     }
     if (!b_last) {
@@ -1049,7 +1050,7 @@
     const int pieceA = std::min(16, bnA * elem), pieceB = std::min(16, (b_last ? 4 * bnB : bnB) * elem);
     if (!inverse) {
       if (pieceA < 4 || pieceB < 4) return 0;
-      if ((p.coef_off[c] * elem) % 16 || (pb.coef_off[c] * elem) % 16 || (p.slice_coefs * elem) % 16) return 0;
+      if ((p.coef_off[c] * elem) % 16 || (pb.coef_off[c] * elem) % 16 || (p.rec_stride[c] * elem) % 16 || (pb.rec_stride[c] * elem) % 16) return 0;
     } else {
       if ((p.coef_off[c] | pb.coef_off[c] | p.rec_stride[c] | pb.rec_stride[c] | bnA) & 3) return 0;
       if ((bnB & 1) && !(bnB == 1 && b_last && spl_of(fw) == 2)) return 0;
diff --git a/vc2-reference_amd/csrc/vc2hip_internal.h b/vc2-reference_amd/csrc/vc2hip_internal.h
--- a/vc2-reference_amd/csrc/vc2hip_internal.h
+++ b/vc2-reference_amd/csrc/vc2hip_internal.h
@@ -172,6 +172,11 @@
 #define VC2_SKIP(p, bit) false
 #endif
 
+struct HeadSplit {
+  int n[3];
+  long long base[3];
+};
+
 struct PackParams {
   const void *store;
   const int32_t *store_wide;
@@ -203,6 +208,7 @@
   unsigned long long *lookback;
   long long lookback_stride;
   unsigned long long *lens;
+  HeadSplit hs;
 };
 
 constexpr int VC2_BP_MAX = 3;
@@ -213,11 +219,6 @@
   long long base[3][VC2_BP_MAX];
   int ow[3][VC2_BP_MAX], np[3][VC2_BP_MAX];
   int lbsh[3][VC2_BP_MAX], lbsw[3][VC2_BP_MAX];
-};
-
-struct HeadSplit {
-  int n[3];
-  long long base[3];
 };
 
 struct UnpackParams {
@@ -301,6 +302,7 @@
 void vc2_launch_pack(Launcher &L, const PackParams &p, int n_pictures, hipStream_t s);
 int vc2_pack_slices_per_tile(const PackParams &p);
 bool vc2_pack_one_pass_default(const PackParams &p);
+bool vc2_pack16_heads(const PackParams &p, int head[3]);
 void vc2_launch_scan_sizes(Launcher &L, const uint32_t *sizes, uint32_t *offsets,
                            unsigned long long *totals, int n_slices, int n_pictures, hipStream_t s);
 void vc2_launch_compact(Launcher &L, const uint8_t *slots, int slot_bytes, const uint32_t *sizes,
diff --git a/vc2-reference_amd/csrc/vc2hip_pack16.h b/vc2-reference_amd/csrc/vc2hip_pack16.h
--- a/vc2-reference_amd/csrc/vc2hip_pack16.h
+++ b/vc2-reference_amd/csrc/vc2hip_pack16.h
@@ -126,7 +126,7 @@
 
 template <bool WRITE>
 __device__ __forceinline__ int p16_general(const int16_t *src, const int32_t *srcw, int n, int n0, int q, const int *qm, int lane,
-                                        unsigned *img, int bit0, int region_bits, unsigned *err) {
+                                        unsigned *img, int bit0, int region_bits, unsigned *err, int hn = 0, int dh = 0) {
   const int n0_shift = (n0 & (n0 - 1)) == 0 ? 31 - __clz(n0) : -1;
   int base = 0, count = 0;
 #pragma unroll 1
@@ -136,7 +136,7 @@
     if (j < n) {
       const int aq = max(q - qm[band_of_index_fast(j, n0, n0_shift)], 0);
       if (aq > 119) atomicOr(err, VC2_DEVERR_QINDEX);
-      else c = quant_dev(St<int16_t>::load1(src + j, srcw + j), aq);
+      else { const int at = j + (j < hn ? dh : 0); c = quant_dev(St<int16_t>::load1(src + at, srcw + at), aq); }
       nb = svlc_bits(c);
       if (nb > 32) { atomicOr(err, VC2_DEVERR_CODE32); c = 0; nb = 1; }
     }
@@ -178,13 +178,16 @@
   const int body_n = (int)(comp == 0 ? p.lane16[67] : (comp == 1 ? p.lane16[68] : p.lane16[69]));
   const int coff = comp == 0 ? p.comp_off[0] : (comp == 1 ? p.comp_off[1] : p.comp_off[2]);
   const bool has_body = cl < body_n, has_head = cl < head_n;
-  const size_t rec_at = (size_t)pic * p.store_stride + (size_t)(active ? slice : 0) * p.slice_coefs;
+  const size_t pic_at = (size_t)pic * p.store_stride;
+  const size_t rec_at = pic_at + (size_t)(active ? slice : 0) * p.slice_coefs;
   const int16_t *rec = (const int16_t *)p.store + rec_at;
   uint4 w0 = make_uint4(0u, 0u, 0u, 0u), w1 = w0;
   int hv = 0;
   if (active && has_body) { const int16_t *b = rec + coff + head_n + 16 * cl; w0 = *(const uint4 *)b; w1 = *(const uint4 *)(b + 8); }
-  if (active && has_head) hv = rec[coff + cl];
-  const int32_t *hwide = p.store_wide + rec_at + coff + cl;
+  const bool heads = p.hs.n[0] != 0;
+  const int hbase = heads ? (int)(comp == 0 ? p.hs.base[0] : (comp == 1 ? p.hs.base[1] : p.hs.base[2])) : coff;
+  const int hat = (active ? slice : 0) * (heads ? head_n : p.slice_coefs) + hbase + cl;
+  if (active && has_head) hv = ((const int16_t *)p.store + pic_at)[hat];
   const int q = p.qidx[(size_t)pic * p.n_slices + (active ? slice : 0)];
   if (threadIdx.x < P16_LUT_N) lut[threadIdx.x] = lut_e;
   if (threadIdx.x < 128) qt[threadIdx.x] = qt_e;
@@ -216,7 +219,7 @@
   int hbits = 0;
   bool hnz = false;
   if (has_head) {
-    if (hv == VC2_ST_SENTINEL) hv = *hwide;
+    if (hv == VC2_ST_SENTINEL) hv = (p.store_wide + pic_at)[hat];
     const int t = quant_core(hv, (int)qh.z, qh.x, (int)qh.y);
     slow |= (unsigned)(t + 65534) > 2u * 65534u;
     hcode = svlc_code(t);
@@ -271,10 +274,11 @@
   const bool slow_any = __any(slow);
   if (__builtin_expect(slow_any, 0)) {
     const int32_t *recw = p.store_wide + rec_at;
+    auto head_dh = [&](int cc) -> int { return p.hs.n[cc] ? (int)p.hs.base[cc] + slice * p.hs.n[cc] - (slice * p.slice_coefs + p.comp_off[cc]) : 0; };
     if constexpr (LB) {
 #pragma unroll 1
       for (int cc = 0; cc < 3; ++cc)
-        bytes[cc] = comp_len(p16_general<false>(rec + p.comp_off[cc], recw + p.comp_off[cc], p.comp_n[cc], p.comp_n0[cc], q, p.qmatrix, lane, nullptr, 0, 0, p.err));
+        bytes[cc] = comp_len(p16_general<false>(rec + p.comp_off[cc], recw + p.comp_off[cc], p.comp_n[cc], p.comp_n0[cc], q, p.qmatrix, lane, nullptr, 0, 0, p.err, p.hs.n[cc], head_dh(cc)));
       lb_publish(p.prefix + 4 + bytes[0] + bytes[1] + bytes[2]);
     }
     int base = p.prefix + 1;
@@ -282,11 +286,11 @@
       const int16_t *src = rec + p.comp_off[cc];
       const int32_t *srcw = recw + p.comp_off[cc];
       if constexpr (!LB) {
-        const int count = p16_general<false>(src, srcw, p.comp_n[cc], p.comp_n0[cc], q, p.qmatrix, lane, nullptr, 0, 0, p.err);
+        const int count = p16_general<false>(src, srcw, p.comp_n[cc], p.comp_n0[cc], q, p.qmatrix, lane, nullptr, 0, 0, p.err, p.hs.n[cc], head_dh(cc));
         bytes[cc] = comp_len(count);
         if (cc == 2) bytes[2] = cbr_v(bytes[2]);
       }
-      p16_general<true>(src, srcw, p.comp_n[cc], p.comp_n0[cc], q, p.qmatrix, lane, wimg, 8 * (wb + base + 1), 8 * bytes[cc], p.err);
+      p16_general<true>(src, srcw, p.comp_n[cc], p.comp_n0[cc], q, p.qmatrix, lane, wimg, 8 * (wb + base + 1), 8 * bytes[cc], p.err, p.hs.n[cc], head_dh(cc));
       if (lane == 0) put_byte(wimg, wb + base, (unsigned)(bytes[cc] / p.scalar));
       base += 1 + bytes[cc];
     }
diff --git a/vc2-reference_amd/csrc/vc2hip_slices.hip b/vc2-reference_amd/csrc/vc2hip_slices.hip
--- a/vc2-reference_amd/csrc/vc2hip_slices.hip
+++ b/vc2-reference_amd/csrc/vc2hip_slices.hip
@@ -754,6 +754,14 @@
   p.lookback = &dummy;
   p.tile_slices = 0;
   return pack16_plan(p, p.lane16);
+}
+bool vc2_pack16_heads(const PackParams &p0, int head[3]) {
+  static const int use16 = vc2_tune_int("VC2HIP_PACK16", 1);
+  if (!use16 || vc2_pack_image_mode(p0.prefix, p0.scalar) != 0) return false;
+  PackParams p = p0;
+  if (!pack16_plan(p, p.lane16)) return false;
+  for (int c = 0; c < 3; ++c) head[c] = (int)p.lane16[64 + c];
+  return true;
 }
 void vc2_launch_pack(Launcher &L, const PackParams &p0, int n_pictures, hipStream_t s) {
   PackParams p = p0;
diff --git a/vc2-reference_amd/vc2hip_py.py b/vc2-reference_amd/vc2hip_py.py
--- a/vc2-reference_amd/vc2hip_py.py
+++ b/vc2-reference_amd/vc2hip_py.py
@@ -12,7 +12,8 @@
 
 FLAGS = {"STORE32": 0x001, "NO_STREAM": 0x002, "NO_PAIR": 0x004, "NO_BANDPLANES": 0x008, "NO_HEADS": 0x010, "NO_CBR_INDEX": 0x020,
          "GENERIC_DWT": 0x040, "SINGLE_PASS_VBR": 0x080, "CBR_GENERAL": 0x100, "LD_DIAGONALS": 0x200,
-         "PLANES8_ALWAYS": 0x400, "PLANES8_NEVER": 0x800, "TWO_PASS_VBR": 0x1000, "CAP_GENERAL": 0x2000}
+         "PLANES8_ALWAYS": 0x400, "PLANES8_NEVER": 0x800, "TWO_PASS_VBR": 0x1000, "CAP_GENERAL": 0x2000,
+         "NO_FWD_HEADS": 0x4000}
 
 KERNELS = {"DD97": 0, "LeGall": 1, "DD137": 2, "Haar0": 3, "Haar1": 4, "Fidelity": 5, "Daub97": 6}
 CF = {"444": 0, "422": 1, "420": 2}
@@ -79,7 +80,7 @@
     "vc2hip_decode_picture_ld", "vc2hip_encode_batch_dev", "vc2hip_decode_batch_dev",
     "vc2hip_profile_enable", "vc2hip_profile_only", "vc2hip_profile_count", "vc2hip_profile_get", "vc2hip_profile_reset",
     "vc2hip_host_alloc", "vc2hip_host_free", "vc2hip_encode_picture_begin", "vc2hip_encode_picture_end",
-    "vc2hip_decode_picture_begin", "vc2hip_decode_picture_end", "vc2hip_band_plane_bits", "vc2hip_dwt_launches",
+    "vc2hip_decode_picture_begin", "vc2hip_decode_picture_end", "vc2hip_band_plane_bits", "vc2hip_forward_heads", "vc2hip_dwt_launches",
     "vc2hip_picture_header", "vc2hip_stream_write_dev", "vc2hip_stream_read_dev",
     "vc2hip_encode_fields_batch_dev", "vc2hip_decode_fields_batch_dev", "vc2hip_decode_reduced_batch_dev",
     "vc2hip_encode_recon_batch_dev", "vc2hip_stream_write_fragments_dev",
@@ -169,6 +170,7 @@
                                        C.POINTER(C.c_double)]
     lib.vc2hip_profile_reset.argtypes = [vp]
     lib.vc2hip_band_plane_bits.argtypes = [vp]
+    lib.vc2hip_forward_heads.argtypes = [vp]
     lib.vc2hip_dwt_launches.argtypes = [vp, C.POINTER(DwtLaunch), C.c_int]
     lib.vc2hip_host_alloc.argtypes = [C.c_size_t]
     lib.vc2hip_host_alloc.restype = vp
@@ -581,6 +583,9 @@
     def band_plane_bits(self):
         return int(self.lib.vc2hip_band_plane_bits(self.h))
 
+    def forward_heads(self):
+        return int(self.lib.vc2hip_forward_heads(self.h))
+
     def dwt_launches(self):
         n = self.lib.vc2hip_dwt_launches(self.h, None, 0)
         self._chk(min(n, 0))
```

New measurement: 125,100 Mpixels/s, median of 6. 1.01x the previous value.
